# TonyLianLong/LLM-groundedDiffusion

Hardware: AMD Instinct MI355X
Metric: images/sec (50-step SD1.5 512^2, LMD+ guidance) (higher is better)
Workload: dtype fp16

## Files before the change

include/lgd_hip.h:

```cpp
#ifndef LGD_HIP_H
#define LGD_HIP_H
#include <stdint.h>
#ifdef __cplusplus
extern "C" {
#endif

#define LGD_ABI_VERSION 12
int lgd_abi_version(void);
int lgd_set_option(const char* name, int value);

#define LGD_EPI_GEGLU 1
#define LGD_EPI_OUT_F32 2
#define LGD_EPI_RES_F32 4
#define LGD_EPI_ROWNORM 8

typedef struct LgdGemmDesc {
  const void* a0;
  const void* a1;
  int64_t lda0, lda1;
  int32_t c0, c1;
  int32_t taps;
  int32_t hin, win, hout, wout, stride, ups;
  const void* w;
  int64_t ldw;
  int32_t M, N, K;
  int32_t nb_o, nb_i;
  int64_t a_bs_o, a_bs_i, w_bs_o, w_bs_i, c_bs_o, c_bs_i, r_bs_o, r_bs_i;
  const float* bias;
  const float* bias2;
  const void* res;
  int64_t ldr;
  float alpha;
  int32_t epi;
  void* c;
  int64_t ldc;
  int32_t splits;
  float* ws;
  int32_t tile;
  int32_t* cnt;
  const float* rowstat;
  const float* colsum;
} LgdGemmDesc;

int lgd_gemm_f16(const LgdGemmDesc* desc , void* stream);
int lgd_gemm_check(const LgdGemmDesc* desc );

int lgd_conv_in_f16(const float* x_nchw, const void* w, const float* bias, void* y, int B, int Cin,
                    int L, int Cout, void* stream);
int lgd_conv_out_f16(const void* x, const void* w, const float* bias, float* y_nchw, int B, int Cin,
                     int L, int Cout, float out_scale, void* stream);

int lgd_groupnorm_f16(const void* x0, const void* x1, int c0, int c1, int B, int HW, int G,
                      float eps, const float* gamma, const float* beta, int silu, void* y,
                      float* part, int nchunk, float* stats, void* stream);
int lgd_groupnorm_bwd_f16(const void* gy, const void* x0, const void* x1, int c0, int c1, int B,
                          int HW, int G, const float* gamma, const float* beta, int silu,
                          const float* stats, void* gx0, void* gx1, float* part, int nchunk,
                          int accumulate, void* stream);

int lgd_layernorm_f16(const void* x, int64_t ldx, void* y, int64_t ldy, int rows, int C, float eps,
                      const float* gamma, const float* beta, float* stats, int rows_per_batch,
                      int64_t x_bs, int64_t y_bs, void* stream);
int lgd_layernorm_bwd_f16(const void* gy, int64_t ldgy, const void* x, int64_t ldx, void* gx,
                          int64_t ldgx, int rows, int C, const float* gamma, const float* stats,
                          int rows_per_batch, int64_t gy_bs, int64_t x_bs, int64_t gx_bs,
                          int accumulate, void* stream);

int lgd_attn_fwd_f16(const void* q, int64_t ldq, int64_t q_bs, const void* k, int64_t ldk,
                     int64_t k_bs, const void* v, int64_t ldv, int64_t v_bs, void* o, int64_t ldo,
                     int64_t o_bs, float* lse, int B, int H, int Sq, int Sk, int d, float scale,
                     void* stream);
int lgd_attn_bwd_f16(const void* q, int64_t ldq, int64_t q_bs, const void* k, int64_t ldk,
                     int64_t k_bs, const void* v, int64_t ldv, int64_t v_bs, const void* o,
                     int64_t ldo, int64_t o_bs, const void* go, int64_t ldgo, int64_t go_bs,
                     const float* lse, float* delta, void* gq, int64_t ldgq, int64_t gq_bs, void* gk,
                     int64_t ldgk, int64_t gk_bs, void* gv, int64_t ldgv, int64_t gv_bs, int B, int H,
                     int Sq, int Sk, int d, float scale, void* stream);
int lgd_attn_bwd_keys_f16(const void* q, int64_t ldq, int64_t q_bs, const void* k, int64_t ldk,
                          int64_t k_bs, const void* v, int64_t ldv, int64_t v_bs, const void* o,
                          int64_t ldo, int64_t o_bs, const void* go, int64_t ldgo, int64_t go_bs,
                          const float* lse, float* delta, void* gq, int64_t ldgq, int64_t gq_bs, void* gk,
                          int64_t ldgk, int64_t gk_bs, void* gv, int64_t ldgv, int64_t gv_bs, int B, int H,
                          int Sq, int Sk, int Sk_grad, int d, float scale, void* stream);

int lgd_cross_attn_fwd_f16(const void* q, int64_t ldq, int64_t q_bs, const void* k, int64_t ldk,
                           int64_t k_bs, const void* v, int64_t ldv, int64_t v_bs, void* o,
                           int64_t ldo, int64_t o_bs, float* probs, int tok, int cond_only, int B,
                           int H, int Sq, int Sk, int d, float scale, void* stream);
int lgd_cross_attn_bwd_f16(const void* q, int64_t ldq, int64_t q_bs, const void* k, int64_t ldk,
                           int64_t k_bs, const void* v, int64_t ldv, int64_t v_bs, const void* go,
                           int64_t ldgo, int64_t go_bs, const float* gp, void* gq, int64_t ldgq,
                           int64_t gq_bs, int B, int H, int Sq, int Sk, int d, float scale,
                           void* stream);

int lgd_attn_causal_fwd_f16(const void* q, int64_t ldq, int64_t q_bs, const void* k, int64_t ldk, int64_t k_bs,
                            const void* v, int64_t ldv, int64_t v_bs, void* o, int64_t ldo, int64_t o_bs, int B,
                            int H, int S, int d, float scale, void* stream);

int lgd_geglu_bwd_f16(const void* h, const void* gy, void* gh, int64_t rows, int n, void* stream);
int lgd_geglu_fwd_f16(const void* h, void* y, int64_t rows, int n, void* stream);
int lgd_quick_gelu_f16(const void* x, void* y, int64_t n, void* stream);
int lgd_nchw_to_nhwc8_f16(const float* x, void* y, int B, int C, int HW, void* stream);
int lgd_add_f16(const void* a, const void* b, void* y, int64_t n, void* stream);
int lgd_scale_f16(const void* x, void* y, float alpha, int64_t n, void* stream);
int lgd_softmax_rows_f16(const void* x, void* y, int64_t rows, int n, float scale, void* stream);
int lgd_upsample2x_bwd_f16(const void* gy, void* gx, int B, int H, int W, int C, void* stream);

int lgd_cfg_ddim_step_f32(const float* eps, const float* x, float* x_out, const float* coef_table,
                          const int32_t* dyn, const float* frozen_ref, const float* mask, float* hist,
                          int B, int C, int HW, void* stream);
int lgd_cfg_multistep_step_f32(const float* eps, const float* x, float* x_out, float* x0_prev,
                               const float* coef_table, const int32_t* dyn, const float* frozen_ref,
                               const float* mask, float* hist, int B, int C, int HW, void* stream);
int lgd_cfg_plms_step_f32(const float* eps, const float* x, float* x_out, float* ets, float* cur_sample,
                          const float* coef_table, const int32_t* dyn, float* hist, int B, int C, int HW, void* stream);
int lgd_scale_rows_f32(const float* x, float* out, const float* table, const int32_t* dyn, int row_stride, int col,
                       int64_t n, int reps, void* stream);
int lgd_axpy_f32(const float* g, float* x, const float* coef_table, const int32_t* step_idx, int col,
                 const float* active, int64_t per_sample, int64_t n, void* stream);
int lgd_select_row_f32(const float* table, const int32_t* idx, float* out, int n, void* stream);

#define LGD_ACT_GELU 1
#define LGD_ACT_RELU 2
int lgd_act_f16(const void* x, void* y, int64_t n, int mode, void* stream);
int lgd_sam_relpos_qkv_f16(const void* qkv, const float* qkv_bias, const float* rel_h, const float* rel_w, int B,
                           int Hs, int Ws, int window, int NH, int d, int DA, float scale, void* qa, void* ka,
                           void* va, void* stream);
int lgd_sam_window_merge_f16(const void* oa, void* out, int B, int Hs, int Ws, int window, int NH, int d, int DA,
                             void* stream);

int lgd_ca_energy_f32(const float* const* maps, float* const* gmaps, const int32_t* map_hw,
                      const int32_t* items, const float* coefs, const float* masks, const float* refs,
                      int64_t refs_step_stride, const int32_t* dyn, const int32_t* groups, int n_groups,
                      int n_items, int n_samples, int H, int T, int max_hw, float grad_scale, float* partial,
                      float* loss, void* stream);

int lgd_boxdiff_energy_f32(const float* const* maps, float* const* gmaps, int n_maps, int side, const int32_t* items,
                           const float* masks, const float* smooth, const int32_t* groups, int n_samples,
                           int max_items, int H, int T, float loss_scale, float grad_scale, float* loss, void* stream);

#ifdef __cplusplus
}
#endif
#endif
```

llm-groundeddiffusion_amd/_lib.py:

```python
import ctypes as C
import os

import torch

_HERE = os.path.dirname(os.path.abspath(__file__))
LIB_PATH = os.path.join(_HERE, "liblgd_hip.so")
ABI_VERSION = 12

c_void_p, c_int, c_i64, c_float = C.c_void_p, C.c_int, C.c_int64, C.c_float


class LgdGemmDesc(C.Structure):
    _fields_ = [
        ("a0", c_void_p), ("a1", c_void_p),
        ("lda0", c_i64), ("lda1", c_i64),
        ("c0", C.c_int32), ("c1", C.c_int32),
        ("taps", C.c_int32),
        ("hin", C.c_int32), ("win", C.c_int32), ("hout", C.c_int32), ("wout", C.c_int32),
        ("stride", C.c_int32), ("ups", C.c_int32),
        ("w", c_void_p), ("ldw", c_i64),
        ("M", C.c_int32), ("N", C.c_int32), ("K", C.c_int32),
        ("nb_o", C.c_int32), ("nb_i", C.c_int32),
        ("a_bs_o", c_i64), ("a_bs_i", c_i64), ("w_bs_o", c_i64), ("w_bs_i", c_i64),
        ("c_bs_o", c_i64), ("c_bs_i", c_i64), ("r_bs_o", c_i64), ("r_bs_i", c_i64),
        ("bias", c_void_p), ("bias2", c_void_p),
        ("res", c_void_p), ("ldr", c_i64),
        ("alpha", c_float), ("epi", C.c_int32),
        ("c", c_void_p), ("ldc", c_i64),
        ("splits", C.c_int32), ("ws", c_void_p),
        ("tile", C.c_int32),
        ("cnt", c_void_p),
        ("rowstat", c_void_p), ("colsum", c_void_p),
    ]


EPI_GEGLU, EPI_OUT_F32, EPI_RES_F32, EPI_ROWNORM = 1, 2, 4, 8

_P, _I, _L, _F = c_void_p, c_int, c_i64, c_float
SIGNATURES = {
    "lgd_abi_version": [],
    "lgd_set_option": [C.c_char_p, _I],
    "lgd_gemm_f16": [C.POINTER(LgdGemmDesc), _P],
    "lgd_gemm_check": [C.POINTER(LgdGemmDesc)],
    "lgd_conv_in_f16": [_P, _P, _P, _P, _I, _I, _I, _I, _P],
    "lgd_conv_out_f16": [_P, _P, _P, _P, _I, _I, _I, _I, _F, _P],
    "lgd_groupnorm_f16": [_P, _P, _I, _I, _I, _I, _I, _F, _P, _P, _I, _P, _P, _I, _P, _P],
    "lgd_groupnorm_bwd_f16": [_P, _P, _P, _I, _I, _I, _I, _I, _P, _P, _I, _P, _P, _P, _P, _I, _I, _P],
    "lgd_layernorm_f16": [_P, _L, _P, _L, _I, _I, _F, _P, _P, _P, _I, _L, _L, _P],
    "lgd_layernorm_bwd_f16": [_P, _L, _P, _L, _P, _L, _I, _I, _P, _P, _I, _L, _L, _L, _I, _P],
    "lgd_attn_fwd_f16": [_P, _L, _L, _P, _L, _L, _P, _L, _L, _P, _L, _L, _P, _I, _I, _I, _I, _I, _F, _P],
    "lgd_attn_bwd_f16": [_P, _L, _L, _P, _L, _L, _P, _L, _L, _P, _L, _L, _P, _L, _L, _P, _P,
                         _P, _L, _L, _P, _L, _L, _P, _L, _L, _I, _I, _I, _I, _I, _F, _P],
    "lgd_attn_bwd_keys_f16": [_P, _L, _L, _P, _L, _L, _P, _L, _L, _P, _L, _L, _P, _L, _L, _P, _P,
                              _P, _L, _L, _P, _L, _L, _P, _L, _L, _I, _I, _I, _I, _I, _I, _F, _P],
    "lgd_cross_attn_fwd_f16": [_P, _L, _L, _P, _L, _L, _P, _L, _L, _P, _L, _L, _P, _I, _I,
                               _I, _I, _I, _I, _I, _F, _P],
    "lgd_cross_attn_bwd_f16": [_P, _L, _L, _P, _L, _L, _P, _L, _L, _P, _L, _L, _P, _P, _L, _L,
                               _I, _I, _I, _I, _I, _F, _P],
    "lgd_geglu_bwd_f16": [_P, _P, _P, _L, _I, _P],
    "lgd_geglu_fwd_f16": [_P, _P, _L, _I, _P],
    "lgd_add_f16": [_P, _P, _P, _L, _P],
    "lgd_softmax_rows_f16": [_P, _P, _L, _I, _F, _P],
    "lgd_scale_f16": [_P, _P, _F, _L, _P],
    "lgd_upsample2x_bwd_f16": [_P, _P, _I, _I, _I, _I, _P],
    "lgd_cfg_ddim_step_f32": [_P, _P, _P, _P, _P, _P, _P, _P, _I, _I, _I, _P],
    "lgd_cfg_multistep_step_f32": [_P, _P, _P, _P, _P, _P, _P, _P, _P, _I, _I, _I, _P],
    "lgd_cfg_plms_step_f32": [_P, _P, _P, _P, _P, _P, _P, _P, _I, _I, _I, _P],
    "lgd_axpy_f32": [_P, _P, _P, _P, _I, _P, _L, _L, _P],
    "lgd_select_row_f32": [_P, _P, _P, _I, _P],
    "lgd_scale_rows_f32": [_P, _P, _P, _P, _I, _I, _L, _I, _P],
    "lgd_attn_causal_fwd_f16": [_P, _L, _L, _P, _L, _L, _P, _L, _L, _P, _L, _L, _I, _I, _I, _I, _F, _P],
    "lgd_quick_gelu_f16": [_P, _P, _L, _P],
    "lgd_act_f16": [_P, _P, _L, _I, _P],
    "lgd_nchw_to_nhwc8_f16": [_P, _P, _I, _I, _I, _P],
    "lgd_sam_relpos_qkv_f16": [_P, _P, _P, _P, _I, _I, _I, _I, _I, _I, _I, _F, _P, _P, _P, _P],
    "lgd_sam_window_merge_f16": [_P, _P, _I, _I, _I, _I, _I, _I, _I, _P],
    "lgd_ca_energy_f32": [_P, _P, _P, _P, _P, _P, _P, _L, _P, _P, _I, _I, _I, _I, _I, _I, _F, _P, _P, _P],
    "lgd_boxdiff_energy_f32": [_P, _P, _I, _I, _P, _P, _P, _P, _I, _I, _I, _I, _F, _F, _P, _P],
}

_lib = None


def load():
    global _lib
    if _lib is not None:
        return _lib
    if not os.path.exists(LIB_PATH):
        raise RuntimeError(
            f"{LIB_PATH} not found: build it with `python __graft_entry__.py` "
            "(there is no CPU/PyTorch fallback for the HIP kernels)")
    lib = C.CDLL(LIB_PATH)
    for name, argtypes in SIGNATURES.items():
        try:
            fn = getattr(lib, name)
        except AttributeError as e:
            raise RuntimeError(f"liblgd_hip.so does not export {name}") from e
        fn.argtypes = argtypes
        fn.restype = c_int
    if lib.lgd_abi_version() != ABI_VERSION:
        raise RuntimeError("liblgd_hip.so ABI version mismatch; rebuild")
    for item in filter(None, os.environ.get("LGD_OPTIONS", "").split(",")):
        name, _, value = item.partition("=")
        check(lib.lgd_set_option(name.strip().encode(), int(value)), f"lgd_set_option({name})")
    _lib = lib
    return lib


_ERR = {-1: "invalid argument", -2: "kernel launch failed", -3: "unsupported shape"}


def check(rc, name):
    if rc != 0:
        raise RuntimeError(f"{name} failed: {_ERR.get(rc, rc)}")
```

llm-groundeddiffusion_amd/csrc/attn.hip:

```cpp
#include <atomic>
#include "common.h"
#include "../../include/lgd_hip.h"
#include "attn_w4.h"
#include <stdlib.h>
#include <string.h>

namespace {

int g_attn32_nw = -1;
int attn32_nw() {
  if (g_attn32_nw < 0) { const char* e = getenv("LGD_ATTN32_NW"); g_attn32_nw = e ? atoi(e) : 8; }
  return g_attn32_nw;
}
int g_attn32_var = 0;
int attn32_var() { return g_attn32_var; }
int g_attn32 = -1;
int attn32_mode() {
  if (g_attn32 < 0) { const char* e = getenv("LGD_ATTN32"); g_attn32 = e ? atoi(e) : 1; }
  return g_attn32;
}

std::atomic<int> g_attn_w4{-1};
int attn_w4_mode() {
  int v = g_attn_w4.load(std::memory_order_relaxed);
// ... 791 lines not shown
    __syncthreads();
    if (t + 2 < n_tiles) load_k((t + 2) * KV_T);
    if (more) load_v((t + 1) * KV_T);
    const float mx_nxt = pipelined_tile((t + 1) & 1, t & 1, s_cur, s_nxt);
    if (more) {
      const float mx = mx_nxt;
      if (__builtin_amdgcn_ballot_w64(mx > 8.f) != 0) {
        const float m_new = (float)(half_t)fmaxf(m_ref, mx + m_ref);
        const float shift = m_new - m_ref;
        const float alpha = __builtin_amdgcn_exp2f(-shift);
#pragma unroll
        for (int dt = 0; dt < NDT; ++dt)
#pragma unroll
          for (int r = 0; r < 16; ++r) oacc[dt][r] *= alpha;
#pragma unroll
        for (int kb = 0; kb < 2; ++kb)
#pragma unroll
          for (int r = 0; r < 16; ++r) s_nxt[kb][r] -= shift;
        m_ref = m_new;
        set_ref(m_new);
      }
#pragma unroll
      for (int kb = 0; kb < 2; ++kb) s_cur[kb] = s_nxt[kb];
    }
  }

  float l;
  {
    const int dl = d & 31, dt_l = d >> 5, h_l = (dl >> 2) & 1, r_l = (dl & 3) + 4 * (dl >> 3);
    float lv = 0.f;
#pragma unroll
    for (int dt = 0; dt < NDT; ++dt)
#pragma unroll
      for (int r = 0; r < 16; ++r)
        if (dt == dt_l && r == r_l) lv = oacc[dt][r];
    l = __shfl(lv, h_l * 32 + qi, 64);
  }
  const int qrow = q0 + qi;
  if (qrow < a.Sq) {
    const float inv = 1.f / l;
    half_t* orow = a.o + (long)b * a.o_bs + (long)qrow * a.ldo + (long)h * d;
#pragma unroll
    for (int dt = 0; dt < NDT; ++dt)
#pragma unroll
      for (int g4 = 0; g4 < 4; ++g4) {
        const int dv = dt * 32 + g4 * 8 + hh * 4;
        if (dv < d) {
          half4_t o;
#pragma unroll
          for (int r = 0; r < 4; ++r) o[r] = (half_t)(oacc[dt][g4 * 4 + r] * inv);
          *reinterpret_cast<half4_t*>(orow + dv) = o;
        }
      }
    if (a.lse && hh == 0) a.lse[((long)b * a.H + h) * a.Sq + qrow] = m_ref + log2f(l);
  }
}

template <int DP, bool SAVE_P>
void launch_attn_dp(const AttnArgs& a, hipStream_t st) {
  if constexpr (SAVE_P) {
    dim3 grid((a.Sq + 63) / 64, a.H, a.B);
    hipLaunchKernelGGL((attn_fwd_kernel<DP>), grid, dim3(256), 0, st, a);
  } else {
    if constexpr (DP == 64 || DP == 96) {
      const int a32 = attn32_mode();
      const int dk = ((a.d + 2 + 15) / 16) * 16;
      const long blocks256 = (long)((a.Sq + 255) / 256) * a.H * a.B;
      if (a32 && a.d % 8 == 0 && (a32 == 2 || (dk == 96 && blocks256 >= 128))) {
        const int var = attn32_var();
        auto go = [&](auto kern, int nw) {
          dim3 g32((a.Sq + 32 * nw - 1) / (32 * nw), a.H, a.B);
          hipLaunchKernelGGL(kern, g32, dim3(64 * nw), 0, st, a);
        };
        if (attn32_nw() == 4 || (a32 != 2 && blocks256 < 256)) {
          if (dk == 48) { go(&attn_self32_kernel<48, 2, 4>, 4); return; }
          if (dk == 96) { go(&attn_self32_kernel<96, 3, 4>, 4); return; }
        } else if (var == 1) {
          if (dk == 48) { go(&attn_self32_kernel<48, 2, 8, 4, true>, 8); return; }
          if (dk == 96) { go(&attn_self32_kernel<96, 3, 8, 4, true>, 8); return; }
        } else if (var == 2) {
          if (dk == 48) { go(&attn_self32_kernel<48, 2, 8, 2, false>, 8); return; }
          if (dk == 96) { go(&attn_self32_kernel<96, 3, 8, 2, false>, 8); return; }
        } else {
          if (dk == 48) { go(&attn_self32_kernel<48, 2, 8>, 8); return; }
          if (dk == 96) { go(&attn_self32_kernel<96, 3, 8>, 8); return; }
        }
      }
    }
    const bool qt2 = (long)((a.Sq + 127) / 128) * a.H * a.B >= 1024 && DP <= 96;
    dim3 grid(qt2 ? (a.Sq + 127) / 128 : (a.Sq + 63) / 64, a.H, a.B);
    if constexpr (DP <= 96) {
      static const int nw_env = [] { const char* e = getenv("LGD_ATTN_NW"); return e ? atoi(e) : 0; }();
      const bool nw8 = nw_env ? nw_env == 8 : ((DP == 64 && a.d < 48) || DP == 96);
      if (qt2 && nw8 && (long)((a.Sq + 255) / 256) * a.H * a.B >= 512) {
        dim3 g8((a.Sq + 255) / 256, a.H, a.B);
        if (DP == 64 && a.d < 48) hipLaunchKernelGGL((attn_self_kernel<DP, true, 2, DP == 64 ? 3 : DP / 16, 8>), g8, dim3(512), 0, st, a);
        else if (a.d < DP) hipLaunchKernelGGL((attn_self_kernel<DP, true, 2, DP / 16, 8>), g8, dim3(512), 0, st, a);
        else hipLaunchKernelGGL((attn_self_kernel<DP, false, 2, DP / 16, 8>), g8, dim3(512), 0, st, a);
        return;
      }
      if (qt2) {
        if (DP == 64 && a.d < 48) hipLaunchKernelGGL((attn_self_kernel<DP, true, 2, DP == 64 ? 3 : DP / 16>), grid, dim3(256), 0, st, a);
        else if (a.d < DP) hipLaunchKernelGGL((attn_self_kernel<DP, true, 2>), grid, dim3(256), 0, st, a);
        else hipLaunchKernelGGL((attn_self_kernel<DP, false, 2>), grid, dim3(256), 0, st, a);
        return;
      }
    }
    if constexpr (DP == 160) {
      static const int wide = [] { const char* e = getenv("LGD_ATTN160"); return e ? atoi(e) : 1; }();
      if (wide && a.d == DP && a.Sq >= 256 && (long)a.H * a.B * ((a.Sq + 63) / 64) > 256) {
        dim3 g8((a.Sq + 255) / 256, a.H, a.B);
        hipLaunchKernelGGL((attn_self_kernel<DP, false, 2, DP / 16, 8>), g8, dim3(512), 0, st, a);
        return;
      }
    }
    if (DP == 64 && a.d < 48) hipLaunchKernelGGL((attn_self_kernel<DP, true, 1, DP == 64 ? 3 : DP / 16>), grid, dim3(256), 0, st, a);
    else if (a.d < DP) hipLaunchKernelGGL((attn_self_kernel<DP, true, 1>), grid, dim3(256), 0, st, a);
    else hipLaunchKernelGGL((attn_self_kernel<DP, false, 1>), grid, dim3(256), 0, st, a);
  }
}

template <bool SAVE_P>
int launch_attn(const AttnArgs& a, hipStream_t st) {
  const int d = a.d;
  if constexpr (!SAVE_P) {
    const int w4 = attn_w4_mode();
    if (w4 && d == 40) {
      AttnW4Args w;
      w.q = a.q; w.ldq = a.ldq; w.q_bs = a.q_bs; w.k = a.k; w.ldk = a.ldk; w.k_bs = a.k_bs;
      w.v = a.v; w.ldv = a.ldv; w.v_bs = a.v_bs; w.o = a.o; w.ldo = a.ldo; w.o_bs = a.o_bs; w.lse = a.lse;
      w.B = a.B; w.H = a.H; w.Sq = a.Sq; w.Sk = a.Sk; w.d = a.d; w.scale_log2 = a.scale_log2;
      const long wgs = (long)((a.Sq + 255) / 256) * a.H * a.B;
      if (lgd_attn_w4_supported(w) && (w4 == 2 || (wgs >= 256 && a.Sk >= 256))) return lgd_attn_w4_launch(w, st);
    }
  }
  if (d <= 32) launch_attn_dp<32, SAVE_P>(a, st);
  else if (d <= 64) launch_attn_dp<64, SAVE_P>(a, st);
  else if (d <= 96) launch_attn_dp<96, SAVE_P>(a, st);
  else if (d <= 128) launch_attn_dp<128, SAVE_P>(a, st);
  else if (d <= 160) launch_attn_dp<160, SAVE_P>(a, st);
  else if (d <= 192) launch_attn_dp<192, SAVE_P>(a, st);
  else return LGD_ERR_UNSUPPORTED;
  return lgd_check_launch();
}

bool bad_view(int64_t ld, int d) { return (ld % 8) != 0 || (d % 8) != 0; }

}

void lgd_gn_set_fused_hw(int hw);
void lgd_gn_set_slab(int on);
void lgd_ln_set_stream(int on);
void lgd_gn_set_apply_wgs(int n);

extern "C" int lgd_set_option(const char* name, int value) {
  if (!name) return LGD_ERR_ARG;
  if (!strcmp(name, "gn_fused") && value >= 0 && value <= 4096) { lgd_gn_set_fused_hw(value); return LGD_OK; }
  if (!strcmp(name, "gn_slab") && (value == 0 || value == 1)) { lgd_gn_set_slab(value); return LGD_OK; }
  if (!strcmp(name, "ln_stream") && (value == 0 || value == 1)) { lgd_ln_set_stream(value); return LGD_OK; }
  if (!strcmp(name, "gn_apply_wgs") && value >= 64 && value <= 8192) { lgd_gn_set_apply_wgs(value); return LGD_OK; }
  if (!strcmp(name, "attn32")) { g_attn32 = value; return LGD_OK; }
  if (!strcmp(name, "attn_w4") && value >= 0 && value <= 2) { g_attn_w4.store(value, std::memory_order_relaxed); return LGD_OK; }
  if (!strcmp(name, "attn_w4_pipe") && (value == 0 || value == 1)) { lgd_attn_w4_set_pipe(value); return LGD_OK; }
  if (!strcmp(name, "attn32_nw") && (value == 4 || value == 8)) { g_attn32_nw = value; return LGD_OK; }
  if (!strcmp(name, "attn32_var") && value >= 0 && value <= 2) { g_attn32_var = value; return LGD_OK; }
  return LGD_ERR_ARG;
}

extern "C" int lgd_attn_fwd_f16(const void* q, int64_t ldq, int64_t q_bs, const void* k,
                                int64_t ldk, int64_t k_bs, const void* v, int64_t ldv, int64_t v_bs,
                                void* o, int64_t ldo, int64_t o_bs, float* lse, int B, int H, int Sq,
                                int Sk, int d, float scale, void* stream) {
  (void)hipGetLastError();
  if (B < 1 || H < 1 || Sq < 1 || Sk < 1 || d < 8) return LGD_ERR_ARG;
  if (bad_view(ldq, d) || bad_view(ldk, d) || bad_view(ldv, d) || (ldo % 4)) return LGD_ERR_ARG;
  AttnArgs a;
  a.q = (const half_t*)q; a.ldq = ldq; a.q_bs = q_bs;
  a.k = (const half_t*)k; a.ldk = ldk; a.k_bs = k_bs;
  a.v = (const half_t*)v; a.ldv = ldv; a.v_bs = v_bs;
  a.o = (half_t*)o; a.ldo = ldo; a.o_bs = o_bs;
  a.lse = lse; a.probs = nullptr; a.tok = -1; a.cond_only = 0; a.causal = 0;
  a.B = B; a.H = H; a.Sq = Sq; a.Sk = Sk; a.d = d;
  a.scale_log2 = scale * 1.4426950408889634f;
  return launch_attn<false>(a, reinterpret_cast<hipStream_t>(stream));
}

extern "C" int lgd_cross_attn_fwd_f16(const void* q, int64_t ldq, int64_t q_bs, const void* k,
                                      int64_t ldk, int64_t k_bs, const void* v, int64_t ldv,
                                      int64_t v_bs, void* o, int64_t ldo, int64_t o_bs, float* probs,
                                      int tok, int cond_only, int B, int H, int Sq, int Sk, int d,
                                      float scale, void* stream) {
  (void)hipGetLastError();
  if (B < 1 || H < 1 || Sq < 1 || Sk < 1 || d < 8) return LGD_ERR_ARG;
  if (bad_view(ldq, d) || bad_view(ldk, d) || bad_view(ldv, d) || (ldo % 4)) return LGD_ERR_ARG;
  if (cond_only && (B % 2)) return LGD_ERR_ARG;
  if (tok >= Sk) return LGD_ERR_ARG;
  AttnArgs a;
  a.q = (const half_t*)q; a.ldq = ldq; a.q_bs = q_bs;
  a.k = (const half_t*)k; a.ldk = ldk; a.k_bs = k_bs;
  a.v = (const half_t*)v; a.ldv = ldv; a.v_bs = v_bs;
  a.o = (half_t*)o; a.ldo = ldo; a.o_bs = o_bs;
  a.lse = nullptr; a.probs = probs; a.tok = tok; a.cond_only = cond_only; a.causal = 0;
  a.B = B; a.H = H; a.Sq = Sq; a.Sk = Sk; a.d = d;
  a.scale_log2 = scale * 1.4426950408889634f;
  hipStream_t st = reinterpret_cast<hipStream_t>(stream);
  if (probs) return launch_attn<true>(a, st);
  return launch_attn<false>(a, st);
}

extern "C" int lgd_attn_causal_fwd_f16(const void* q, int64_t ldq, int64_t q_bs, const void* k, int64_t ldk,
                                       int64_t k_bs, const void* v, int64_t ldv, int64_t v_bs, void* o,
                                       int64_t ldo, int64_t o_bs, int B, int H, int S, int d, float scale,
                                       void* stream) {
  (void)hipGetLastError();
  if (B < 1 || H < 1 || S < 1 || d < 8) return LGD_ERR_ARG;
  if (bad_view(ldq, d) || bad_view(ldk, d) || bad_view(ldv, d) || (ldo % 4)) return LGD_ERR_ARG;
  AttnArgs a;
  a.q = (const half_t*)q; a.ldq = ldq; a.q_bs = q_bs;
  a.k = (const half_t*)k; a.ldk = ldk; a.k_bs = k_bs;
  a.v = (const half_t*)v; a.ldv = ldv; a.v_bs = v_bs;
  a.o = (half_t*)o; a.ldo = ldo; a.o_bs = o_bs;
  a.lse = nullptr; a.probs = nullptr; a.tok = -1; a.cond_only = 0; a.causal = 1;
  a.B = B; a.H = H; a.Sq = S; a.Sk = S; a.d = d;
  a.scale_log2 = scale * 1.4426950408889634f;
  return launch_attn<true>(a, reinterpret_cast<hipStream_t>(stream));
}
```

llm-groundeddiffusion_amd/csrc/gemm.hip:

```cpp
#include "common.h"
#include "../../include/lgd_hip.h"
#include <map>
#include <mutex>
#include <utility>
#include <stdlib.h>

namespace {

constexpr int BK = 64;
constexpr int LDS_LD = BK + 16;

struct GemmArgs {
  LgdGemmDesc d;
  int cin;
  int k_per_split;
  int group_m;
#ifdef LGD_GEMM_ABLATION
  int stagger;
#endif
};

__device__ __forceinline__ float4 ld_bias4(const float* p, int n) {
  return *reinterpret_cast<const float4*>(p + n);
}

__device__ __forceinline__ f32x4 rownorm4(const LgdGemmDesc& d, int m, int n_in, f32x4 v) {
  if (d.epi & LGD_EPI_ROWNORM) {
    const float2 st = *reinterpret_cast<const float2*>(d.rowstat + (long)m * 2);
    const float4 cs = *reinterpret_cast<const float4*>(d.colsum + n_in);
    v[0] = st.y * (v[0] - st.x * cs.x); v[1] = st.y * (v[1] - st.x * cs.y);
    v[2] = st.y * (v[2] - st.x * cs.z); v[3] = st.y * (v[3] - st.x * cs.w);
  }
  return v;
}

template <bool GEGLU>
__device__ __forceinline__ f32x4 epilogue_value4(const LgdGemmDesc& d, long r_off, int m, int n_out, f32x4 v, f32x4 g,
                                                 float4 bv, float4 bg, bool res_ready, half4_t res_pre) {
  v[0] += bv.x; v[1] += bv.y; v[2] += bv.z; v[3] += bv.w;
  if (GEGLU) {
    g[0] += bg.x; g[1] += bg.y; g[2] += bg.z; g[3] += bg.w;
#ifdef LGD_GEMM_ABLATION
    if (d.epi & (1 << 16)) {
#pragma unroll
      for (int r = 0; r < 4; ++r) v[r] = v[r] * g[r];
    } else
#endif
    {
      const f32x2_t g01 = gelu2_f((f32x2_t){g[0], g[1]}), g23 = gelu2_f((f32x2_t){g[2], g[3]});
      v[0] *= g01[0]; v[1] *= g01[1]; v[2] *= g23[0]; v[3] *= g23[1];
    }
  }
  const float alpha = d.alpha;
#pragma unroll
  for (int r = 0; r < 4; ++r) v[r] *= alpha;
  if (res_ready) {
#pragma unroll
    for (int r = 0; r < 4; ++r) v[r] += (float)res_pre[r];
  } else if (d.res) {
    if (d.epi & LGD_EPI_RES_F32) {
      const float* rp = reinterpret_cast<const float*>(d.res) + r_off + (long)m * d.ldr + n_out;
      float4 rv = *reinterpret_cast<const float4*>(rp);
      v[0] += rv.x; v[1] += rv.y; v[2] += rv.z; v[3] += rv.w;
    } else {
      const half_t* rp = reinterpret_cast<const half_t*>(d.res) + r_off + (long)m * d.ldr + n_out;
      half4_t rv = *reinterpret_cast<const half4_t*>(rp);
#pragma unroll
      for (int r = 0; r < 4; ++r) v[r] += (float)rv[r];
    }
  }
  return v;
}

template <bool GEGLU>
__device__ __forceinline__ void epilogue_store4(const LgdGemmDesc& d, long c_off, long r_off, int m,
                                                int n_out, f32x4 v, f32x4 g, float4 bv, float4 bg,
                                                bool res_ready = false,
                                                half4_t res_pre = (half4_t){0, 0, 0, 0}) {
  v = epilogue_value4<GEGLU>(d, r_off, m, n_out, v, g, bv, bg, res_ready, res_pre);
  if (d.epi & LGD_EPI_OUT_F32) {
    float* cp = reinterpret_cast<float*>(d.c) + c_off + (long)m * d.ldc + n_out;
    *reinterpret_cast<float4*>(cp) = make_float4(v[0], v[1], v[2], v[3]);
  } else {
    half_t* cp = reinterpret_cast<half_t*>(d.c) + c_off + (long)m * d.ldc + n_out;
    half4_t o;
#pragma unroll
    for (int r = 0; r < 4; ++r) o[r] = (half_t)v[r];
    *reinterpret_cast<half4_t*>(cp) = o;
  }
}

__device__ __forceinline__ float4 ld_bias_sum4(const LgdGemmDesc& d, int n) {
  float4 b = make_float4(0.f, 0.f, 0.f, 0.f);
  if (d.bias) b = ld_bias4(d.bias, n);
  if (d.bias2) {
    float4 b2 = ld_bias4(d.bias2, n);
    b.x += b2.x; b.y += b2.y; b.z += b2.z; b.w += b2.w;
  }
  return b;
}

template <int MI, int NI>
__device__ __forceinline__ void gemm_epilogue(const GemmArgs& ga, f32x4 (&acc)[NI][MI], int m0, int n0,
                                              int wm, int wn, int lane, int batch, int split,
                                              long c_off, long r_off, int* lds_flag = nullptr) {
  const LgdGemmDesc& d = ga.d;
  const int m_l = lane & 15;
  const int n_l = (lane >> 4) * 4;
  if (d.splits > 1) {
    float* ws = ga.d.ws + ((long)batch * d.splits + split) * (long)d.M * d.N;
#pragma unroll
    for (int mi = 0; mi < MI; ++mi) {
      int m = m0 + wm * 16 * MI + mi * 16 + m_l;
      if (m >= d.M) continue;
#pragma unroll
      for (int ni = 0; ni < NI; ++ni) {
        int n = n0 + wn * 16 * NI + ni * 16 + n_l;
        if (n >= d.N) continue;
        f32x4 v = acc[ni][mi];
        *reinterpret_cast<float4*>(ws + (long)m * d.N + n) = make_float4(v[0], v[1], v[2], v[3]);
      }
    }
    if (!d.cnt || !lds_flag) return;
    asm volatile("s_waitcnt vmcnt(0)" ::: "memory");
    __syncthreads();
    int32_t* cnt = d.cnt + (long)batch * gridDim.x + blockIdx.x;
    if (threadIdx.x == 0) {
      __builtin_amdgcn_fence(__ATOMIC_RELEASE, "agent");
      asm volatile("s_waitcnt vmcnt(0)" ::: "memory");
      *lds_flag = __hip_atomic_fetch_add(cnt, 1, __ATOMIC_RELAXED, __HIP_MEMORY_SCOPE_AGENT);
    }
    __syncthreads();
    if (*lds_flag != d.splits - 1) return;
    if (threadIdx.x == 0) {
      __builtin_amdgcn_fence(__ATOMIC_ACQUIRE, "agent");
      __hip_atomic_store(cnt, 0, __ATOMIC_RELAXED, __HIP_MEMORY_SCOPE_AGENT);
    }
    __syncthreads();
    const float* w0 = ga.d.ws + (long)batch * d.splits * (long)d.M * d.N;
#pragma unroll
    for (int mi = 0; mi < MI; ++mi) {
      const int m = m0 + wm * 16 * MI + mi * 16 + m_l;
#pragma unroll
      for (int ni = 0; ni < NI; ++ni) {
        const int n = n0 + wn * 16 * NI + ni * 16 + n_l;
        f32x4 v = {0.f, 0.f, 0.f, 0.f};
        if (m < d.M && n < d.N) {
          for (int s2 = 0; s2 < d.splits; ++s2) {
            const float4 t = *reinterpret_cast<const float4*>(w0 + (long)s2 * d.M * d.N + (long)m * d.N + n);
            v[0] += t.x; v[1] += t.y; v[2] += t.z; v[3] += t.w;
          }
        }
        acc[ni][mi] = v;
      }
    }
  }
  const bool geglu = d.epi & LGD_EPI_GEGLU;
  if (geglu) {
    if constexpr (NI % 2 == 0) {
#pragma unroll
      for (int ni = 0; ni < NI; ni += 2) {
        const int n_in = n0 + wn * 16 * NI + ni * 16 + n_l;
        if (n_in >= d.N) continue;
        const int n_out = (n0 + wn * 16 * NI + ni * 16) / 2 + n_l;
        const float4 bv = ld_bias_sum4(d, n_in);
        float4 bg = make_float4(0.f, 0.f, 0.f, 0.f);
        if (d.bias) bg = ld_bias4(d.bias, n_in + 16);
#pragma unroll
        for (int mi = 0; mi < MI; ++mi) {
// ... 14 lines not shown
    half4_t rpre[NCH][MI];
    if (res16) {
      const half_t* rb = reinterpret_cast<const half_t*>(d.res) + r_off;
#pragma unroll
      for (int nj = 0; nj < NCH; ++nj) {
        int n = n0 + wn * 16 * NI + (nc + nj) * 16 + n_l;
        if (n >= d.N) n = 0;
#pragma unroll
        for (int mi = 0; mi < MI; ++mi) {
          int m = m0 + wm * 16 * MI + mi * 16 + m_l;
          if (m >= d.M) m = d.M - 1;
          rpre[nj][mi] = *reinterpret_cast<const half4_t*>(rb + (long)m * d.ldr + n);
        }
      }
    }
#pragma unroll
    for (int nj = 0; nj < NCH; ++nj) {
      const int ni = nc + nj;
      const int n = n0 + wn * 16 * NI + ni * 16 + n_l;
      if (n >= d.N) continue;
      const float4 bv = ld_bias_sum4(d, n);
#pragma unroll
      for (int mi = 0; mi < MI; ++mi) {
        const int m = m0 + wm * 16 * MI + mi * 16 + m_l;
        if (m < d.M)
          epilogue_store4<false>(d, c_off, r_off, m, n, rownorm4(d, m, n, acc[ni][mi]), acc[ni][mi], bv, bv, res16,
                                 res16 ? rpre[nj][mi] : (half4_t){0, 0, 0, 0});
      }
    }
  }
}

template <int MI, int NI, int WM, int WN, int STAGE_B, bool GEGLU, bool RES_PREFETCH>
__device__ __forceinline__ void gemm_epilogue_lds_generic(const GemmArgs& ga, f32x4 (&acc)[NI][MI], int m0, int n0, int wm,
                                                  int wn, int lane, int tid, long c_off, long r_off,
                                                  unsigned char* lds) {
  const LgdGemmDesc& d = ga.d;
  constexpr int NT = 64 * WM * WN;
  constexpr int BM = WM * 16 * MI, BN = WN * 16 * NI;
  constexpr int BN_OUT = GEGLU ? BN / 2 : BN;
  constexpr int NI_OUT = GEGLU ? NI / 2 : NI;
  constexpr int CROW = BN_OUT * 2 + 16;
  constexpr int R = (BM * CROW <= STAGE_B) ? 1 : ((BM / 2) * CROW <= STAGE_B) ? 2 : 4;
  static_assert(MI % R == 0 && (BM / R) * CROW <= STAGE_B, "staged rows must fit one ring stage");
  constexpr int MI_R = MI / R;
  constexpr int WROWS = 16 * MI_R;
  constexpr int RROWS = WM * WROWS;
  constexpr int CPR = BN_OUT / 8;
  const int m_l = lane & 15, n_l = (lane >> 4) * 4;
  const int n0_out = GEGLU ? n0 / 2 : n0;
  const int n_total_out = GEGLU ? d.N / 2 : d.N;
  const bool res16 = d.res && !(d.epi & LGD_EPI_RES_F32);
  half_t* cbase = reinterpret_cast<half_t*>(d.c) + c_off;
  float4 bv[NI_OUT], bg[NI_OUT];
  const bool rn = d.epi & LGD_EPI_ROWNORM;
  float4 cv[NI_OUT], cg[NI_OUT];
  float2 st[MI];
#pragma unroll
  for (int no = 0; no < NI_OUT; ++no) {
    const int n_out = n0_out + wn * 16 * NI_OUT + no * 16 + n_l;
    const int n_in = GEGLU ? n0 + wn * 16 * NI + no * 32 + n_l : n_out;
    bv[no] = make_float4(0.f, 0.f, 0.f, 0.f);
    bg[no] = bv[no];
    cv[no] = bv[no];
    cg[no] = bv[no];
#ifdef LGD_GEMM_ABLATION
    if (d.epi & (1 << 18)) continue;
#endif
    if (n_out < n_total_out) {
      bv[no] = ld_bias_sum4(d, n_in);
      if (GEGLU && d.bias) bg[no] = ld_bias4(d.bias, n_in + 16);
      if (rn) {
        cv[no] = *reinterpret_cast<const float4*>(d.colsum + n_in);
        if (GEGLU) cg[no] = *reinterpret_cast<const float4*>(d.colsum + n_in + 16);
      }
    }
  }
#pragma unroll
  for (int mi = 0; mi < MI; ++mi) {
    int m = m0 + wm * 16 * MI + mi * 16 + m_l;
    if (m >= d.M) m = d.M - 1;
    st[mi] = rn ? *reinterpret_cast<const float2*>(d.rowstat + (long)m * 2) : make_float2(0.f, 1.f);
  }
  auto rownorm = [&](f32x4 v, const float2 s2, const float4 c) {
    if (rn) {
      v[0] = s2.y * (v[0] - s2.x * c.x); v[1] = s2.y * (v[1] - s2.x * c.y);
      v[2] = s2.y * (v[2] - s2.x * c.z); v[3] = s2.y * (v[3] - s2.x * c.w);
    }
    return v;
  };
#pragma unroll
  for (int r = 0; r < R; ++r) {
    half4_t rpre[NI_OUT][MI_R];
    if (res16 && !GEGLU) {
      const half_t* rb = reinterpret_cast<const half_t*>(d.res) + r_off;
#pragma unroll
      for (int no = 0; no < NI_OUT; ++no) {
        int n = n0_out + wn * 16 * NI_OUT + no * 16 + n_l;
        if (n >= n_total_out) n = 0;
#pragma unroll
        for (int mj = 0; mj < MI_R; ++mj) {
          int m = m0 + wm * 16 * MI + (r * MI_R + mj) * 16 + m_l;
          if (m >= d.M) m = d.M - 1;
          rpre[no][mj] = *reinterpret_cast<const half4_t*>(rb + (long)m * d.ldr + n);
        }
      }
    }
#pragma unroll
    for (int no = 0; no < NI_OUT; ++no) {
      const int n_out = n0_out + wn * 16 * NI_OUT + no * 16 + n_l;
      const int nn = n_out < n_total_out ? n_out : 0;
#pragma unroll
      for (int mj = 0; mj < MI_R; ++mj) {
        const int mi = r * MI_R + mj;
        int m = m0 + wm * 16 * MI + mi * 16 + m_l;
        if (m >= d.M) m = d.M - 1;
        f32x4 v;
        if constexpr (GEGLU) {
          v = epilogue_value4<true>(d, r_off, m, nn, rownorm(acc[2 * no][mi], st[mi], cv[no]), rownorm(acc[2 * no + 1][mi], st[mi], cg[no]),
                                    bv[no], bg[no], false, (half4_t){0, 0, 0, 0});
        } else {
          v = epilogue_value4<false>(d, r_off, m, nn, rownorm(acc[no][mi], st[mi], cv[no]), acc[no][mi], bv[no], bv[no], res16,
                                     res16 ? rpre[no][mj] : (half4_t){0, 0, 0, 0});
        }
        half4_t o;
#pragma unroll
        for (int e = 0; e < 4; ++e) o[e] = (half_t)v[e];
        *reinterpret_cast<half4_t*>(lds + (wm * WROWS + mj * 16 + m_l) * CROW + (wn * 16 * NI_OUT + no * 16 + n_l) * 2) = o;
      }
    }
    asm volatile("s_waitcnt lgkmcnt(0)" ::: "memory");
    __builtin_amdgcn_s_barrier();
#pragma unroll
    for (int i = 0; i < (RROWS * CPR + NT - 1) / NT; ++i) {
      const int idx = tid + i * NT;
      const int row = idx / CPR, ch = idx - row * CPR;
      const int wr = row / WROWS;
      const int m = m0 + wr * 16 * MI + r * WROWS + (row - wr * WROWS), n = n0_out + ch * 8;
#ifdef LGD_GEMM_ABLATION
      if ((d.epi & (1 << 17)) && idx != 0) continue;
#endif
      if (idx < RROWS * CPR && m < d.M && n < n_total_out) {
        const uint4 val = *reinterpret_cast<const uint4*>(lds + row * CROW + ch * 16);
        *reinterpret_cast<uint4*>(cbase + (long)m * d.ldc + n) = val;
      }
    }
    if (r + 1 < R || !RES_PREFETCH) {
      asm volatile("s_waitcnt lgkmcnt(0)" ::: "memory");
      __builtin_amdgcn_s_barrier();
    }
  }
}

template <int MI, int NI, int WM, int WN, int STAGE_B, bool GEGLU, bool RES_PREFETCH, bool RES16, bool RN>
__device__ __forceinline__ void gemm_epilogue_lds(const GemmArgs& ga, f32x4 (&acc)[NI][MI], int m0, int n0, int wm,
                                                  int wn, int lane, int tid, long c_off, long r_off,
                                                  unsigned char* lds) {
  static_assert(!(GEGLU && RES16), "GEGLU outputs take no residual here");
  const LgdGemmDesc& d = ga.d;
  constexpr int NT = 64 * WM * WN;
  constexpr int BM = WM * 16 * MI, BN = WN * 16 * NI;
  constexpr int BN_OUT = GEGLU ? BN / 2 : BN;
  constexpr int NI_OUT = GEGLU ? NI / 2 : NI;
  constexpr int CROW = BN_OUT * 2 + 16;
  constexpr int R = (BM * CROW <= STAGE_B) ? 1 : ((BM / 2) * CROW <= STAGE_B) ? 2 : 4;
  static_assert(MI % R == 0 && (BM / R) * CROW <= STAGE_B, "staged rows must fit one ring stage");
  constexpr int MI_R = MI / R;
  constexpr int WROWS = 16 * MI_R;
  constexpr int RROWS = WM * WROWS;
  constexpr int CPR = BN_OUT / 8;
  const int m_l = lane & 15, n_l = (lane >> 4) * 4;
  const int n0_out = GEGLU ? n0 / 2 : n0;
  const int n_total_out = GEGLU ? d.N / 2 : d.N;
  half_t* cbase = reinterpret_cast<half_t*>(d.c) + c_off;
  const f32x2_t alpha2 = {d.alpha, d.alpha};
  constexpr bool LEAN = MI * NI >= 32;
  constexpr bool LEAN2 = MI * NI >= 32 && WN == 4;
  float4 bv[NI_OUT], bg[NI_OUT], cv[NI_OUT], cg[NI_OUT];
  int ncol[NI_OUT];
#pragma unroll
  for (int no = 0; no < NI_OUT; ++no) {
    const int n_out = n0_out + wn * 16 * NI_OUT + no * 16 + n_l;
    const int n_in = GEGLU ? n0 + wn * 16 * NI + no * 32 + n_l : n_out;
    const bool ok = n_out < n_total_out;
    ncol[no] = ok ? n_out : 0;
    bv[no] = make_float4(0.f, 0.f, 0.f, 0.f);
    bg[no] = bv[no];
    cv[no] = bv[no];
    cg[no] = bv[no];
#ifdef LGD_GEMM_ABLATION
    if (d.epi & (1 << 18)) continue;
#endif
    if (ok && !LEAN2) {
      bv[no] = ld_bias_sum4(d, n_in);
      if (GEGLU && d.bias) bg[no] = ld_bias4(d.bias, n_in + 16);
      if constexpr (RN && !LEAN) {
        cv[no] = *reinterpret_cast<const float4*>(d.colsum + n_in);
        if (GEGLU) cg[no] = *reinterpret_cast<const float4*>(d.colsum + n_in + 16);
      }
    }
  }
  int mrow[MI];
  float2 st[MI];
#pragma unroll
  for (int mi = 0; mi < MI; ++mi) {
    int m = m0 + wm * 16 * MI + mi * 16 + m_l;
    if (m >= d.M) m = d.M - 1;
    mrow[mi] = m;
    st[mi] = make_float2(0.f, 1.f);
    if constexpr (RN && !LEAN2) st[mi] = *reinterpret_cast<const float2*>(d.rowstat + (long)m * 2);
  }
  auto normed = [&](const f32x4& v, const float2 s2, const float4 c, const float4 b, f32x2_t& lo, f32x2_t& hi) {
    lo = (f32x2_t){v[0], v[1]};
    hi = (f32x2_t){v[2], v[3]};
    if constexpr (RN) {
      const f32x2_t mean = {s2.x, s2.x}, rstd = {s2.y, s2.y};
      lo = rstd * (lo - mean * (f32x2_t){c.x, c.y});
      hi = rstd * (hi - mean * (f32x2_t){c.z, c.w});
    }
    lo += (f32x2_t){b.x, b.y};
    hi += (f32x2_t){b.z, b.w};
  };
  unsigned char* lw = lds + (wm * WROWS + m_l) * CROW + (wn * 16 * NI_OUT + n_l) * 2;
#pragma unroll
  for (int r = 0; r < R; ++r) {
    if constexpr (RN && LEAN2) {
#pragma unroll
      for (int mj = 0; mj < MI_R; ++mj)
        st[r * MI_R + mj] = *reinterpret_cast<const float2*>(d.rowstat + (long)mrow[r * MI_R + mj] * 2);
    }
    half4_t rpre[NI_OUT][MI_R];
    if constexpr (RES16) {
      const half_t* rb = reinterpret_cast<const half_t*>(d.res) + r_off;
#pragma unroll
      for (int mj = 0; mj < MI_R; ++mj) {
        const half_t* rrow = rb + (long)mrow[r * MI_R + mj] * d.ldr;
#pragma unroll
        for (int no = 0; no < NI_OUT; ++no) {
          int nc = ncol[no];
          if constexpr (LEAN) {
            const int n_out = n0_out + wn * 16 * NI_OUT + no * 16 + n_l;
            nc = n_out < n_total_out ? n_out : 0;
          }
          rpre[no][mj] = *reinterpret_cast<const half4_t*>(rrow + nc);
        }
      }
    }
#pragma unroll
    for (int no = 0; no < NI_OUT; ++no) {
      if constexpr ((RN && LEAN) || LEAN2) {
        const int n_out = n0_out + wn * 16 * NI_OUT + no * 16 + n_l;
        const int n_in = GEGLU ? n0 + wn * 16 * NI + no * 32 + n_l : n_out;
        if (n_out < n_total_out) {
          if constexpr (RN) {
            cv[no] = *reinterpret_cast<const float4*>(d.colsum + n_in);
            if (GEGLU) cg[no] = *reinterpret_cast<const float4*>(d.colsum + n_in + 16);
          }
          if constexpr (LEAN2) {
            bv[no] = ld_bias_sum4(d, n_in);
            if (GEGLU && d.bias) bg[no] = ld_bias4(d.bias, n_in + 16);
          }
        }
      }
#pragma unroll
      for (int mj = 0; mj < MI_R; ++mj) {
        const int mi = r * MI_R + mj;
        f32x2_t lo, hi;
        if constexpr (GEGLU) {
          f32x2_t glo, ghi;
          normed(acc[2 * no][mi], st[mi], cv[no], bv[no], lo, hi);
          normed(acc[2 * no + 1][mi], st[mi], cg[no], bg[no], glo, ghi);
#ifdef LGD_GEMM_ABLATION
          if (d.epi & (1 << 16)) { lo *= glo; hi *= ghi; } else
#endif
          { lo *= gelu2_f(glo); hi *= gelu2_f(ghi); }
        } else {
          normed(acc[no][mi], st[mi], cv[no], bv[no], lo, hi);
        }
        lo *= alpha2;
        hi *= alpha2;
        if constexpr (RES16) {
          const half4_t rr = rpre[no][mj];
          lo += (f32x2_t){(float)rr[0], (float)rr[1]};
          hi += (f32x2_t){(float)rr[2], (float)rr[3]};
        }
        const half4_t o = {(half_t)lo[0], (half_t)lo[1], (half_t)hi[0], (half_t)hi[1]};
        *reinterpret_cast<half4_t*>(lw + mj * 16 * CROW + no * 32) = o;
      }
    }
    asm volatile("s_waitcnt lgkmcnt(0)" ::: "memory");
    __builtin_amdgcn_s_barrier();
#pragma unroll LEAN2 ? 1 : (RROWS * CPR + NT - 1) / NT
    for (int i = 0; i < (RROWS * CPR + NT - 1) / NT; ++i) {
      const int idx = tid + i * NT;
      const int row = idx / CPR, ch = idx - row * CPR;
      const int wr = row / WROWS;
      const int m = m0 + wr * 16 * MI + r * WROWS + (row - wr * WROWS), n = n0_out + ch * 8;
#ifdef LGD_GEMM_ABLATION
      if ((d.epi & (1 << 17)) && idx != 0) continue;
#endif
      if (idx < RROWS * CPR && m < d.M && n < n_total_out) {
        const uint4 val = *reinterpret_cast<const uint4*>(lds + row * CROW + ch * 16);
        *reinterpret_cast<uint4*>(cbase + (long)m * d.ldc + n) = val;
      }
    }
    if (r + 1 < R || !RES_PREFETCH) {
      asm volatile("s_waitcnt lgkmcnt(0)" ::: "memory");
      __builtin_amdgcn_s_barrier();
    }
  }
}

template <int MI, int NI>
__global__ __launch_bounds__(256) void gemm_kernel(const GemmArgs ga) {
  constexpr int BM = 32 * MI;
  constexpr int BN = 32 * NI;
  constexpr int A_IT = BM * 8 / 256;
  constexpr int B_IT = BN * 8 / 256;
  static_assert(A_IT >= 1 && B_IT >= 1, "tile too small");

  __shared__ __attribute__((aligned(16))) half_t smem[(BM + BN) * LDS_LD];
  half_t* As = smem;
  half_t* Bs = smem + BM * LDS_LD;

  const LgdGemmDesc& d = ga.d;
  const int tid = threadIdx.x;
  const int lane = tid & 63;
  const int wid = tid >> 6;
  const int wm = wid >> 1, wn = wid & 1;

  const int n_tiles_n = (d.N + BN - 1) / BN;
  const int tile_m = blockIdx.x / n_tiles_n;
  const int tile_n = blockIdx.x - tile_m * n_tiles_n;
  const int zz = blockIdx.z;
  const int batch = zz / d.splits;
  const int split = zz - batch * d.splits;
  const int b_o = batch / d.nb_i, b_i = batch - b_o * d.nb_i;
  const long a_off = b_o * d.a_bs_o + b_i * d.a_bs_i;
  const long w_off = b_o * d.w_bs_o + b_i * d.w_bs_i;
  const long c_off = b_o * d.c_bs_o + b_i * d.c_bs_i;
  const long r_off = b_o * d.r_bs_o + b_i * d.r_bs_i;

  const int m0 = tile_m * BM, n0 = tile_n * BN;
  const int k_beg = split * ga.k_per_split;
  int k_end = k_beg + ga.k_per_split;
  if (k_end > d.K) k_end = d.K;
  const int nk = (k_end - k_beg + BK - 1) / BK;

  const half_t* A0 = reinterpret_cast<const half_t*>(d.a0) + a_off;
  const half_t* A1 = d.a1 ? reinterpret_cast<const half_t*>(d.a1) + a_off : nullptr;
  const half_t* W = reinterpret_cast<const half_t*>(d.w) + w_off;

  const int kseg = tid & 7;
  const int rbase = tid >> 3;
  const int cin = ga.cin;
  const bool conv = d.taps == 9;

  int a_iy0[A_IT], a_ix0[A_IT];
  long a_row[A_IT];
  bool a_ok[A_IT];
#pragma unroll
  for (int i = 0; i < A_IT; ++i) {
    int m = m0 + rbase + 32 * i;
    a_ok[i] = m < d.M;
    if (conv) {
      int hw = d.hout * d.wout;
      int b = m / hw;
      int rem = m - b * hw;
      int oy = rem / d.wout;
      int ox = rem - oy * d.wout;
      a_iy0[i] = oy * d.stride - 1;
      a_ix0[i] = ox * d.stride - 1;
      a_row[i] = (long)b * d.hin * d.win;
    } else {
      a_iy0[i] = 0; a_ix0[i] = 0;
      a_row[i] = m;
    }
  }
  int k_cur = k_beg + kseg * 8;
  int tap = conv ? k_cur / cin : 0;
  int ch = k_cur - tap * cin;

  uint4 a_reg[A_IT], b_reg[B_IT];

  auto load_tile = [&]() {
    const bool k_ok = k_cur < k_end;
    int ky = 0, kx = 0;
    if (conv) { ky = tap / 3; kx = tap - ky * 3; }
    const bool src1 = ch >= d.c0;
    const half_t* src = src1 ? A1 : A0;
    const long ld = src1 ? d.lda1 : d.lda0;
    const int cc = src1 ? ch - d.c0 : ch;
#pragma unroll
    for (int i = 0; i < A_IT; ++i) {
      bool ok = a_ok[i] && k_ok;
      long row = a_row[i];
      if (conv) {
        int iy = a_iy0[i] + ky, ix = a_ix0[i] + kx;
        if (d.ups) {
          ok = ok && iy >= 0 && ix >= 0 && iy < 2 * d.hin && ix < 2 * d.win;
          if (d.ups == 2) ok = ok && !((iy | ix) & 1);
          iy >>= 1; ix >>= 1;
        } else {
          ok = ok && iy >= 0 && ix >= 0 && iy < d.hin && ix < d.win;
        }
        row += (long)iy * d.win + ix;
      }
      if (ok) a_reg[i] = *reinterpret_cast<const uint4*>(src + row * ld + cc);
      else a_reg[i] = make_uint4(0, 0, 0, 0);
    }
#pragma unroll
    for (int i = 0; i < B_IT; ++i) {
      int n = n0 + rbase + 32 * i;
      bool ok = (n < d.N) && k_ok;
      if (ok) b_reg[i] = *reinterpret_cast<const uint4*>(W + (long)n * d.ldw + k_cur);
      else b_reg[i] = make_uint4(0, 0, 0, 0);
    }
    k_cur += BK;
    ch += BK;
    if (conv) {
      while (ch >= cin) { ch -= cin; ++tap; }
    }
  };
  auto store_tile = [&]() {
#pragma unroll
    for (int i = 0; i < A_IT; ++i)
      *reinterpret_cast<uint4*>(As + (rbase + 32 * i) * LDS_LD + kseg * 8) = a_reg[i];
#pragma unroll
    for (int i = 0; i < B_IT; ++i)
      *reinterpret_cast<uint4*>(Bs + (rbase + 32 * i) * LDS_LD + kseg * 8) = b_reg[i];
  };

  f32x4 acc[NI][MI];
#pragma unroll
  for (int ni = 0; ni < NI; ++ni)
#pragma unroll
    for (int mi = 0; mi < MI; ++mi) acc[ni][mi] = (f32x4){0.f, 0.f, 0.f, 0.f};

  const int frow = lane & 15;
  const int fk = (lane >> 4) * 8;

  if (nk > 0) {
    load_tile();
    store_tile();
    __syncthreads();
    for (int kt = 0; kt < nk; ++kt) {
      if (kt + 1 < nk) load_tile();
#pragma unroll
      for (int kk = 0; kk < BK / 32; ++kk) {
        half8_t af[MI], bf[NI];
#pragma unroll
        for (int mi = 0; mi < MI; ++mi)
          af[mi] = *reinterpret_cast<const half8_t*>(
              As + (wm * 16 * MI + mi * 16 + frow) * LDS_LD + kk * 32 + fk);
#pragma unroll
        for (int ni = 0; ni < NI; ++ni)
          bf[ni] = *reinterpret_cast<const half8_t*>(
              Bs + (wn * 16 * NI + ni * 16 + frow) * LDS_LD + kk * 32 + fk);
#pragma unroll
        for (int ni = 0; ni < NI; ++ni)
#pragma unroll
// ... 440 lines not shown
      else p = (a_ok[j] && live) ? a_ptr[j] : zero;
      __builtin_amdgcn_global_load_lds((glb_ptr_t)p, (lds_ptr_t)(As + (j * NW + wid) * 8 * BK), 16, 0, 0);
    } else {
      const int i = j - A_IT;
      const half_t* p = live ? w_row[i] : zero;
      if (B_HALF && i == B_FULL) {
        if (b_half_on)
          __builtin_amdgcn_global_load_lds((glb_ptr_t)p, (lds_ptr_t)(Bs + b_grp_last * 8 * BK), 16, 0, 0);
      } else {
        __builtin_amdgcn_global_load_lds((glb_ptr_t)p, (lds_ptr_t)(Bs + (i * NW + wid) * 8 * BK), 16, 0, 0);
      }
    }
  };
  auto advance = [&]() {
    ++kt_issue;
    if constexpr (TWO) return;
    if (CM) {
      int wstep = cin;
      if (++tap0 == 9) { tap0 = 0; ch0 += BK; wstep = BK - 8 * cin; }
#pragma unroll
      for (int i = 0; i < B_IT; ++i) w_row[i] += wstep;
      cm_offset();
    } else {
#pragma unroll
      for (int i = 0; i < B_IT; ++i) w_row[i] += BK;
#pragma unroll
      for (int i = 0; i < A_IT; ++i) a_ptr[i] += BK;
      const int prev = ch0;
      ch0 += BK;
      bool red = prev < d.c0 && ch0 >= d.c0;
      if (ch0 >= cin) { ch0 -= cin; ++tap0; red = true; }
      if (red && kt_issue < nk) derive();
    }
  };

  f32x4 acc[NI][MI];
#pragma unroll
  for (int ni = 0; ni < NI; ++ni)
#pragma unroll
    for (int mi = 0; mi < MI; ++mi) acc[ni][mi] = (f32x4){0.f, 0.f, 0.f, 0.f};

  const int frow = lane & 15;
  const int fg = lane >> 4;
  const int fsw = (frow >> 1) & 7;
  const unsigned lds0 = (unsigned)(uintptr_t)smem;
  const unsigned a_b0 = lds0 + ((wm * 16 * MI + frow) * BK + ((0 * 4 + fg) ^ fsw) * 8) * 2;
  const unsigned a_b1 = lds0 + ((wm * 16 * MI + frow) * BK + ((1 * 4 + fg) ^ fsw) * 8) * 2;
  constexpr int B_OFF = BM * BK * 2;
  const unsigned b_b0 = a_b0 - (wm * 16 * MI) * BK * 2 + B_OFF + (wn * 16 * NI) * BK * 2;
  const unsigned b_b1 = a_b1 - (wm * 16 * MI) * BK * 2 + B_OFF + (wn * 16 * NI) * BK * 2;
  using seqA = std::make_integer_sequence<int, MI>;
  using seqB = std::make_integer_sequence<int, NI>;
  constexpr int FSTR = 16 * BK * 2;

  half8_t af0[MI], bf0[NI], af1[MI], bf1[NI];
  auto mma_range = [&](half8_t (&af)[MI], half8_t (&bf)[NI], int g0, int g1) {
#pragma unroll
    for (int g = 0; g < NMMA; ++g)
      if (g >= g0 && g < g1) {
        const int ni = g / MI, mi = g % MI;
        if constexpr (ABL & 4) {
          asm volatile("" : "+v"(acc[ni][mi]) : "v"(bf[ni]), "v"(af[mi]));
        } else {
          acc[ni][mi] = __builtin_amdgcn_mfma_f32_16x16x32_f16(bf[ni], af[mi], acc[ni][mi], 0, 0, 0);
        }
      }
  };
  auto dma_and_mma = [&](int j0, int cnt, unsigned so_b, bool live, half8_t (&af)[MI], half8_t (&bf)[NI]) {
#pragma unroll
    for (int j = 0; j < T_DMA; ++j)
      if (j < cnt) {
        if constexpr (!(ABL & 1)) issue_one(j0 + j, (int)(so_b >> 1), live);
        __builtin_amdgcn_sched_barrier(0);
        mma_range(af, bf, (NMMA * j) / cnt, (NMMA * (j + 1)) / cnt);
        __builtin_amdgcn_sched_barrier(0);
      }
    if (cnt == 0) mma_range(af, bf, 0, NMMA);
  };

  int v_issue = blockIdx.x;
  bool issue_dead = false;
  auto begin_k_tile = [&]() {
    if constexpr (!PERSIST) {
      issue_dead = kt_issue >= nk;
      return;
    }
    if (kt_issue >= nk && !issue_dead) {
      v_issue += gridDim.x;
      if (v_issue < total_tiles) {
        int m0n, n0n;
        tile_origin(v_issue, m0n, n0n);
        setup_issue(m0n, n0n);
        if (CM) cm_offset(); else derive();
      } else {
        issue_dead = true;
      }
    }
  };

  if (nk > 0) {
    int m0, n0;
    tile_origin(blockIdx.x, m0, n0);
    setup_issue(m0, n0);
    if (CM) cm_offset(); else derive();
#pragma unroll
    for (int t = 0; t < D; ++t) {
      begin_k_tile();
#pragma unroll
      for (int j = 0; j < T_DMA; ++j) issue_one(j, t * STAGE, !issue_dead);
      advance();
    }
    asm volatile("s_waitcnt vmcnt(%0)" ::"n"((D - 1) * T_DMA) : "memory");
    __builtin_amdgcn_s_barrier();
    lds_read_frags<0, FSTR>(af0, a_b0, seqA{});
    lds_read_frags<0, FSTR>(bf0, b_b0, seqB{});
    unsigned so_cur = 0, so_nxt = STAGE_B, so_iss = (D % NS) * STAGE_B;
    auto next_stage = [](unsigned x) { x += STAGE_B; return x == NS * STAGE_B ? 0u : x; };
    auto k_loop = [&]() {
      for (int kt = 0; kt < nk; ++kt) {
        begin_k_tile();
        const bool live = !issue_dead;
        wait_frags<-1>(af0, bf0);
        if constexpr (!(ABL & 2)) {
          lds_read_frags<0, FSTR>(af1, a_b1 + so_cur, seqA{});
          lds_read_frags<0, FSTR>(bf1, b_b1 + so_cur, seqB{});
        }
        dma_and_mma(0, T1, so_iss, live, af0, bf0);
        wait_frags<(D - 2) * T_DMA + T1>(af1, bf1);
        if constexpr (!(ABL & 8)) __builtin_amdgcn_s_barrier();
        if constexpr (!(ABL & 2)) {
          if (!PERSIST || kt + 1 < nk) {
            lds_read_frags<0, FSTR>(af0, a_b0 + so_nxt, seqA{});
            lds_read_frags<0, FSTR>(bf0, b_b0 + so_nxt, seqB{});
          }
        }
        dma_and_mma(T1, T2, so_iss, live, af1, bf1);
        advance();
        so_cur = so_nxt; so_nxt = next_stage(so_nxt); so_iss = next_stage(so_iss);
      }
    };
    const bool lds_epi = d.splits == 1 && !(d.epi & LGD_EPI_OUT_F32) && !(d.N & 7) && !(d.ldc & 7) && !(c_off & 7) &&
                         !(reinterpret_cast<uintptr_t>(d.c) & 15) && !((d.epi & LGD_EPI_GEGLU) && (NI & 1)) &&
                         !(d.res && (d.epi & (LGD_EPI_RES_F32 | LGD_EPI_GEGLU)));
    auto epilogue = [&](int m0_, int n0_) {
      if constexpr (ABL & 16) {
#pragma unroll
        for (int ni = 0; ni < NI; ++ni)
#pragma unroll
          for (int mi = 0; mi < MI; ++mi) asm volatile("" ::"v"(acc[ni][mi]));
        return;
      }
      if (lds_epi) {
        unsigned char* free_stage = reinterpret_cast<unsigned char*>(smem) + so_iss;
#define LGD_EPI_LDS(G, RS, RNORM) \
  gemm_epilogue_lds<MI, NI, WM, WN, STAGE_B, G, !PERSIST, RS, RNORM>(ga, acc, m0_, n0_, wm, wn, lane, tid, c_off, r_off, free_stage)
        const bool rn_ = d.epi & LGD_EPI_ROWNORM;
        if constexpr (MI * NI >= 32) {
          if (d.epi & LGD_EPI_GEGLU)
            gemm_epilogue_lds_generic<MI, NI, WM, WN, STAGE_B, true, !PERSIST>(ga, acc, m0_, n0_, wm, wn, lane, tid, c_off, r_off, free_stage);
          else
            gemm_epilogue_lds_generic<MI, NI, WM, WN, STAGE_B, false, !PERSIST>(ga, acc, m0_, n0_, wm, wn, lane, tid, c_off, r_off, free_stage);
        } else if (d.epi & LGD_EPI_GEGLU) {
          if constexpr (NI % 2 == 0) {
            if (rn_) LGD_EPI_LDS(true, false, true); else LGD_EPI_LDS(true, false, false);
          }
        } else if (d.res) {
          if (rn_) LGD_EPI_LDS(false, true, true); else LGD_EPI_LDS(false, true, false);
        } else {
          if (rn_) LGD_EPI_LDS(false, false, true); else LGD_EPI_LDS(false, false, false);
        }
#undef LGD_EPI_LDS
      } else {
        if constexpr (!(TWO && MI * NI >= 32))
          gemm_epilogue<MI, NI>(ga, acc, m0_, n0_, wm, wn, lane, batch, split, c_off, r_off, reinterpret_cast<int*>(smem));
      }
    };
    if constexpr (PERSIST) {
      for (int v = blockIdx.x; v < total_tiles; v += gridDim.x) {
        tile_origin(v, m0, n0);
        k_loop();
        epilogue(m0, n0);
#pragma unroll
        for (int ni = 0; ni < NI; ++ni)
#pragma unroll
          for (int mi = 0; mi < MI; ++mi) acc[ni][mi] = (f32x4){0.f, 0.f, 0.f, 0.f};
        if constexpr (!(ABL & 2)) {
          lds_read_frags<0, FSTR>(af0, a_b0 + so_cur, seqA{});
          lds_read_frags<0, FSTR>(bf0, b_b0 + so_cur, seqB{});
        }
      }
      asm volatile("s_waitcnt vmcnt(0) lgkmcnt(0)" ::: "memory");
    } else {
      k_loop();
      asm volatile("s_waitcnt vmcnt(0) lgkmcnt(0)" ::: "memory");
      epilogue(m0, n0);
    }
  } else {
    for (int v = blockIdx.x; v < total_tiles; v += gridDim.x) {
      int m0, n0;
      tile_origin(v, m0, n0);
      if constexpr (!(TWO && MI * NI >= 32))
        gemm_epilogue<MI, NI>(ga, acc, m0, n0, wm, wn, lane, batch, split, c_off, r_off, reinterpret_cast<int*>(smem));
    }
  }
}

template <int MI, int NI, bool CM, int ABL = 0>
__global__ __launch_bounds__(512, 1) void gemm_phase_kernel(const GemmArgs ga) {
  constexpr int WM = 2, WN = 4;
  static_assert(MI == 8, "128 rows per wave group");
  constexpr int MH = MI / 2;
  constexpr int NI0 = (NI + 1) / 2, NI1 = NI - NI0;
  constexpr int BM = WM * 16 * MI, BN = WN * 16 * NI;
  constexpr int AQ_B = 2 * 16 * MH * 128;
  constexpr int BQ0_B = 64 * NI0 * 128, BQ1_B = 64 * NI1 * 128;
  constexpr int OFF_A1 = AQ_B, OFF_B0 = 2 * AQ_B, OFF_B1 = 2 * AQ_B + BQ0_B;
  constexpr int STAGE_B = 2 * AQ_B + BQ0_B + BQ1_B;
  static_assert(STAGE_B == (BM + BN) * BK * 2 && 2 * STAGE_B <= 160 * 1024, "LDS");
  constexpr int NA = 2;
  constexpr int T_DMA = 2 * NA + NI;
  constexpr unsigned OOB = 0x80000000u;
  constexpr unsigned NREC = 0x80000000u;

  extern __shared__ __attribute__((aligned(1024))) half_t smem[];
  unsigned char* lds = reinterpret_cast<unsigned char*>(smem);

  const LgdGemmDesc& d = ga.d;
  const int tid = threadIdx.x;
  const int lane = tid & 63;
  const int wid = __builtin_amdgcn_readfirstlane(tid >> 6);
  const int grp = wid >> 2, wn = wid & 3;

  const int n_tiles_n = (d.N + BN - 1) / BN;
  const int total_tiles = ((d.M + BM - 1) / BM) * n_tiles_n;
  int m0, n0;
  {
    const int q = total_tiles >> 3, r = total_tiles & 7;
    const int xcd = blockIdx.x & 7, idx = blockIdx.x >> 3;
    const int bid = (xcd < r ? xcd * (q + 1) : r * (q + 1) + (xcd - r) * q) + idx;
    int tile_m, tile_n;
    if (ga.group_m > 1) {
      const int per_group = ga.group_m * n_tiles_n;
      const int g = bid / per_group, in = bid - g * per_group;
      const int n_tiles_m = total_tiles / n_tiles_n;
      int rows = n_tiles_m - g * ga.group_m;
      if (rows > ga.group_m) rows = ga.group_m;
      tile_n = in / rows;
      tile_m = g * ga.group_m + (in - tile_n * rows);
    } else {
      tile_m = bid / n_tiles_n;
      tile_n = bid - tile_m * n_tiles_n;
    }
    m0 = __builtin_amdgcn_readfirstlane(tile_m * BM);
    n0 = __builtin_amdgcn_readfirstlane(tile_n * BN);
  }
  const int split = blockIdx.z;
  constexpr int batch = 0;
  constexpr long a_off = 0, w_off = 0, c_off = 0, r_off = 0;

  const int k_beg = split * ga.k_per_split;
  int k_end = k_beg + ga.k_per_split;
  if (k_end > d.K) k_end = d.K;
  const int nk = __builtin_amdgcn_readfirstlane((k_end - k_beg) / BK);
  const int cin = ga.cin;

  const int lrow = lane >> 3;
  const int kseg = (lane & 7) ^ ((((wid & 1) << 2) + (lrow >> 1)) & 7);
  const unsigned lda2 = (unsigned)d.lda0 * 2u, ldw2 = (unsigned)d.ldw * 2u;
  const int arow = wid * 8 + lrow;
  const int bcol = (wid >> 1) * 16 * NI + (wid & 1) * 8 + lrow;
  const half_t* a_base = reinterpret_cast<const half_t*>(d.a0) + a_off - (CM ? (long)(d.win + 1) * d.lda0 : 0L);
  const half_t* w_base = reinterpret_cast<const half_t*>(d.w) + w_off;
  const unsigned voffA = (unsigned)(m0 + arow) * lda2 + kseg * 16;
  const unsigned voffB = (unsigned)(n0 + bcol) * ldw2 + kseg * 16;
  unsigned amask[2] = {0u, 0u};
#pragma unroll
  for (int h = 0; h < 2; ++h)
#pragma unroll
    for (int j = 0; j < NA; ++j) {
      const int m = m0 + j * 128 + h * 16 * MH + arow;
      if (m >= d.M) continue;
      if (CM) {
        const int ox = m % d.wout, oy = (m / d.wout) % d.hout;
#pragma unroll
        for (int t = 0; t < 9; ++t) {
          const int iy = oy + t / 3 - 1, ix = ox + t % 3 - 1;
          if (iy >= 0 && ix >= 0 && iy < d.hin && ix < d.win) amask[h] |= 1u << (9 * j + t);
        }
      } else {
        amask[h] |= 1u << (9 * j);
      }
    }
  unsigned bmask = 0;
#pragma unroll
  for (int i = 0; i < NI; ++i)
    if (n0 + bcol + i * 16 < d.N) bmask |= 1u << i;

  const int t0 = k_beg / BK;
  auto k_pos = [&](int kt, unsigned& sa, unsigned& sw, int& tap) {
    if (CM) {
      const int t = t0 + kt, ch = __builtin_amdgcn_readfirstlane(t / 9);
      tap = t - ch * 9;
      const int ky = tap / 3, kx = tap - ky * 3;
      sa = (unsigned)(ky * d.win + kx) * lda2 + (unsigned)ch * (BK * 2);
      sw = (unsigned)(tap * cin + ch * BK) * 2u;
    } else {
      tap = 0;
      sa = sw = (unsigned)(k_beg + kt * BK) * 2u;
    }
  };
  auto dma_a = [&](int h, unsigned so, bool live, unsigned sa, int tap, bool inloop = true) {
    if ((ABL & 1) && inloop) return;
    const __amdgpu_buffer_rsrc_t rs = __builtin_amdgcn_make_buffer_rsrc(const_cast<half_t*>(a_base), 0, live ? NREC : 0u, 0x00020000);
#pragma unroll
    for (int j = 0; j < NA; ++j) {
      const unsigned vo = ((amask[h] >> (9 * j + tap)) & 1u) ? voffA : OOB;
      __builtin_amdgcn_raw_ptr_buffer_load_lds(rs, (lds_ptr_t)(lds + so + (h ? OFF_A1 : 0) + (j * 8 + wid) * 1024), 16, vo,
                                               sa + (unsigned)(j * 128 + h * 16 * MH) * lda2, 0, 0);
    }
  };
  auto dma_b = [&](int q, unsigned so, bool live, unsigned sw, bool inloop = true) {
    if ((ABL & 1) && inloop) return;
// ... 88 lines not shown
      LGD_PH_BAR();
      if constexpr (!(ABL & 2)) lds_read_frags<BQ0_B, 64 * 128>(bf1[0], b_ad0, seqB1{});
      if constexpr (!(ABL & 2)) lds_read_frags<BQ0_B, 64 * 128>(bf1[1], b_ad1, seqB1{});
      dma_a(1, so_nxt, live1, sa1, tap1);
      asm volatile("s_waitcnt vmcnt(%0)" ::"n"(T_DMA) : "memory");
      LGD_PH_BAR();
      LGD_PH_MMA(bf1, NI1, NI0, 0);
      LGD_PH_BAR();
      if constexpr (!(ABL & 2)) lds_read_frags<OFF_A1, 16 * 128>(af[0], a_ad0, seqA{});
      if constexpr (!(ABL & 2)) lds_read_frags<OFF_A1, 16 * 128>(af[1], a_ad1, seqA{});
      dma_b(0, so_cur, live2, sw2);
      LGD_PH_BAR();
      LGD_PH_MMA(bf1, NI1, NI0, MH);
      LGD_PH_BAR();
      dma_a(0, so_cur, live2, sa2, tap2);
      asm volatile("s_waitcnt vmcnt(%0)" ::"n"(T_DMA) : "memory");
      LGD_PH_BAR();
      LGD_PH_MMA(bf0, NI0, 0, MH);
      LGD_PH_BAR();
      a_ad0 += sdelta; a_ad1 += sdelta; b_ad0 += sdelta; b_ad1 += sdelta;
      sdelta = -sdelta;
      const unsigned t = so_cur; so_cur = so_nxt; so_nxt = t;
    }
    if (grp == 0 && !(ABL & 64)) LGD_PH_BAR();
    asm volatile("s_waitcnt vmcnt(0) lgkmcnt(0)" ::: "memory");
    LGD_PH_BAR();
  }
  else {
#pragma unroll
    for (int ni = 0; ni < NI; ++ni)
#pragma unroll
      for (int mi = 0; mi < MI; ++mi) acc[ni][mi] = (f32x4){0.f, 0.f, 0.f, 0.f};
  }
#undef LGD_PH_MMA
#undef LGD_PH_BAR

  if constexpr (ABL & 16) {
#pragma unroll
    for (int ni = 0; ni < NI; ++ni)
#pragma unroll
      for (int mi = 0; mi < MI; ++mi) asm volatile("" ::"v"(acc[ni][mi]));
    return;
  }
  if (d.splits > 1) {
    const int m_l = lane & 15, n_l = (lane >> 4) * 4;
    float* ws = d.ws + ((long)batch * d.splits + split) * (long)d.M * d.N;
#pragma unroll
    for (int mi = 0; mi < MI; ++mi) {
      const int m = m0 + grp * 16 * MI + mi * 16 + m_l;
      if (m >= d.M) continue;
#pragma unroll
      for (int ni = 0; ni < NI; ++ni) {
        const int n = n0 + wn * 16 * NI + ni * 16 + n_l;
        if (n >= d.N) continue;
        const f32x4 v = acc[ni][mi];
        *reinterpret_cast<float4*>(ws + (long)m * d.N + n) = make_float4(v[0], v[1], v[2], v[3]);
      }
    }
    return;
  }
#define LGD_EPI_LDS(G, RS, RNORM) \
  gemm_epilogue_lds<MI, NI, WM, WN, (MI * NI > 32 ? STAGE_B : 2 * STAGE_B), G, true, RS, RNORM>(ga, acc, m0, n0, grp, wn, lane, tid, c_off, r_off, lds)
  const bool rn_ = d.epi & LGD_EPI_ROWNORM;
  if (d.epi & LGD_EPI_GEGLU) {
    if constexpr (NI % 2 == 0) {
      if (rn_) LGD_EPI_LDS(true, false, true); else LGD_EPI_LDS(true, false, false);
    }
  } else if (d.res) {
    if (rn_) LGD_EPI_LDS(false, true, true); else LGD_EPI_LDS(false, true, false);
  } else {
    if (rn_) LGD_EPI_LDS(false, false, true); else LGD_EPI_LDS(false, false, false);
  }
#undef LGD_EPI_LDS
}

__global__ __launch_bounds__(256) void splitk_reduce_kernel(const GemmArgs ga) {
  const LgdGemmDesc& d = ga.d;
  const bool geglu = d.epi & LGD_EPI_GEGLU;
  const int n_out_cols = geglu ? d.N / 2 : d.N;
  const long groups_per_row = n_out_cols / 4;
  const long total = (long)d.M * groups_per_row;
  const int batch = blockIdx.z;
  const int b_o = batch / d.nb_i, b_i = batch - b_o * d.nb_i;
  const long c_off = b_o * d.c_bs_o + b_i * d.c_bs_i;
  const long r_off = b_o * d.r_bs_o + b_i * d.r_bs_i;
  const float* ws = d.ws + (long)batch * d.splits * (long)d.M * d.N;
  for (long idx = blockIdx.x * 256L + threadIdx.x; idx < total; idx += (long)gridDim.x * 256L) {
    int m = (int)(idx / groups_per_row);
    int gcol = (int)(idx - (long)m * groups_per_row) * 4;
    int n_in = geglu ? (gcol / 16) * 32 + (gcol % 16) : gcol;
    f32x4 v = {0.f, 0.f, 0.f, 0.f}, g = {0.f, 0.f, 0.f, 0.f};
    for (int s = 0; s < d.splits; ++s) {
      const float* p = ws + (long)s * d.M * d.N + (long)m * d.N + n_in;
      float4 t = *reinterpret_cast<const float4*>(p);
      v[0] += t.x; v[1] += t.y; v[2] += t.z; v[3] += t.w;
      if (geglu) {
        float4 u = *reinterpret_cast<const float4*>(p + 16);
        g[0] += u.x; g[1] += u.y; g[2] += u.z; g[3] += u.w;
      }
    }
    const float4 bv = ld_bias_sum4(d, n_in);
    v = rownorm4(d, m, n_in, v);
    if (geglu) {
      float4 bg = make_float4(0.f, 0.f, 0.f, 0.f);
      if (d.bias) bg = ld_bias4(d.bias, n_in + 16);
      epilogue_store4<true>(d, c_off, r_off, m, gcol, v, rownorm4(d, m, n_in + 16, g), bv, bg);
    } else {
      epilogue_store4<false>(d, c_off, r_off, m, gcol, v, g, bv, bv);
    }
  }
}

enum GemmLoop : int {
  LOOP_REG,
  LOOP_DMA,
  LOOP_DMA8,
  LOOP_PIPE,
  LOOP_PHASE,
};
enum : unsigned {
  TILE_GEGLU = 1,
  TILE_PLAIN = 2,
  TILE_ONE_SPLIT = 4,
  TILE_LDS_EPI = 8,
  TILE_CONV_SAME = 16,
  TILE_CNT = 32,
};
struct GemmTile {
  int code;
  GemmLoop loop;
  int bm, bn;
  unsigned flags;
};
constexpr unsigned TILE_STD = TILE_GEGLU | TILE_CNT;
constexpr GemmTile GEMM_TILES[] = {
    {1, LOOP_REG, 128, 128, TILE_STD},   {2, LOOP_REG, 128, 64, TILE_STD},     {3, LOOP_REG, 64, 128, TILE_STD},
    {4, LOOP_REG, 64, 64, TILE_STD},     {5, LOOP_REG, 32, 128, TILE_STD},     {6, LOOP_REG, 128, 160, TILE_CNT},
    {7, LOOP_REG, 64, 160, TILE_CNT},
    {17, LOOP_DMA, 128, 128, TILE_STD},  {18, LOOP_DMA, 128, 64, TILE_STD},    {19, LOOP_DMA, 64, 128, TILE_STD},
    {20, LOOP_DMA, 64, 64, TILE_STD},    {21, LOOP_DMA, 32, 128, TILE_STD},    {22, LOOP_DMA, 128, 160, TILE_CNT},
    {23, LOOP_DMA, 64, 160, TILE_CNT},
    {25, LOOP_DMA8, 256, 320, TILE_CNT}, {26, LOOP_DMA8, 256, 128, TILE_STD},
    {33, LOOP_PIPE, 256, 160, TILE_CNT}, {34, LOOP_PIPE, 256, 128, TILE_STD}, {35, LOOP_PIPE, 256, 64, TILE_STD},
    {37, LOOP_PIPE, 128, 160, TILE_CNT}, {38, LOOP_PIPE, 128, 128, TILE_STD}, {39, LOOP_PIPE, 128, 64, TILE_STD},
    {40, LOOP_PIPE, 64, 160, TILE_CNT},  {41, LOOP_PIPE, 64, 128, TILE_STD},  {42, LOOP_PIPE, 64, 64, TILE_STD},
    {44, LOOP_PIPE, 256, 256, TILE_GEGLU | TILE_PLAIN | TILE_ONE_SPLIT | TILE_LDS_EPI},
    {45, LOOP_PIPE, 128, 128, TILE_STD | TILE_PLAIN},
    {46, LOOP_PHASE, 256, 256, TILE_GEGLU | TILE_LDS_EPI | TILE_CONV_SAME},
    {47, LOOP_PHASE, 256, 320, TILE_LDS_EPI | TILE_CONV_SAME},
};

const GemmTile* gemm_check(const LgdGemmDesc& desc, GemmArgs& ga) {
  ga.d = desc;
  LgdGemmDesc& d = ga.d;
  if (d.M <= 0 || d.N <= 0 || d.K <= 0) return nullptr;
  if (d.taps != 1 && d.taps != 9) return nullptr;
  ga.cin = d.c0 + d.c1;
  if (d.K != d.taps * ga.cin) return nullptr;
  if ((d.c0 % 8) || (d.c1 % 8) || (d.N % 4) || (d.ldw % 8) || (d.lda0 % 8) || (d.lda1 % 8) ||
      (d.ldc % 4))
    return nullptr;
  if (d.c1 > 0 && !d.a1) return nullptr;
  if (d.res && (d.ldr % 4)) return nullptr;
  if (d.nb_o < 1) d.nb_o = 1;
  if (d.nb_i < 1) d.nb_i = 1;
  if (d.splits < 1) d.splits = 1;
  const bool geglu = d.epi & LGD_EPI_GEGLU;
  if (geglu && (d.N % 32)) return nullptr;
  if (d.splits > 1 && !d.ws) return nullptr;
  if ((d.epi & LGD_EPI_ROWNORM) && (!d.rowstat || !d.colsum || d.taps != 1 || d.nb_o * d.nb_i != 1 || d.c1 > 0))
    return nullptr;
  int ktiles = (d.K + BK - 1) / BK;
  int tps = (ktiles + d.splits - 1) / d.splits;
  ga.k_per_split = tps * BK;
  d.splits = (ktiles + tps - 1) / tps;

  int code = d.tile;
  if (code == 0) {
    long batches = (long)d.nb_o * d.nb_i * d.splits;
    auto wgs = [&](int bm, int bn) {
      return batches * ((d.M + bm - 1) / bm) * ((d.N + bn - 1) / bn);
    };
    if (d.M <= 32) code = 21;
    else if (!geglu && d.N % 160 == 0 && wgs(128, 160) >= 384) code = 22;
    else if (!geglu && d.N % 160 == 0 && wgs(64, 160) >= 256) code = 23;
    else if (wgs(128, 128) >= 384 && d.N % 128 == 0) code = 17;
    else if (wgs(64, 128) >= 256 && d.N % 128 == 0) code = 19;
    else code = 20;
  }
  const GemmTile* t = nullptr;
  for (const GemmTile& e : GEMM_TILES)
    if (e.code == code) t = &e;
  if (!t) return nullptr;
  const unsigned f = t->flags;
  if (geglu && !(f & TILE_GEGLU)) return nullptr;
  if (t->loop == LOOP_DMA8 && (d.K % BK)) return nullptr;
  if ((t->loop == LOOP_PIPE || t->loop == LOOP_PHASE) && ((d.K % BK) || (ga.cin % BK) || (d.c0 % BK))) return nullptr;
  if ((f & TILE_PLAIN) && (d.taps != 1 || d.c1 > 0)) return nullptr;
  if (t->loop == LOOP_PHASE) {
    if (d.c1 > 0 || d.nb_o * d.nb_i != 1) return nullptr;
    if (((long)d.M + 2L * d.win + 2) * d.lda0 * 2 + 2L * d.K >= (1L << 31) || (long)d.N * d.ldw * 2 >= (1L << 31))
      return nullptr;
  }
  if ((f & TILE_CONV_SAME) && d.taps == 9 && (d.stride != 1 || d.ups != 0 || d.hin != d.hout || d.win != d.wout))
    return nullptr;
  if ((f & TILE_ONE_SPLIT) && d.splits != 1) return nullptr;
  if ((f & TILE_LDS_EPI) && d.splits == 1) {
    const long c_off_max = (long)(d.nb_o - 1) * d.c_bs_o + (long)(d.nb_i - 1) * d.c_bs_i;
    if ((d.epi & LGD_EPI_OUT_F32) || (d.N & 7) || (d.ldc & 7) || (c_off_max & 7) || (d.c_bs_o & 7) || (d.c_bs_i & 7) ||
        (reinterpret_cast<uintptr_t>(d.c) & 15) || (d.res && (d.epi & (LGD_EPI_RES_F32 | LGD_EPI_GEGLU))))
      return nullptr;
  }
  if (d.splits > 1 && d.cnt && !(f & TILE_CNT)) return nullptr;
  return t;
}

using GemmKernel = void (*)(GemmArgs);

int lds_kernel(GemmKernel kern, int smem, int threads, long* resident = nullptr) {
  static std::mutex mu;
  static std::map<std::pair<GemmKernel, int>, long> ready;
  int dev = 0;
  if (hipGetDevice(&dev) != hipSuccess) return LGD_ERR_LAUNCH;
  std::lock_guard<std::mutex> lock(mu);
  auto it = ready.find({kern, dev});
  if (it == ready.end()) {
    if (hipFuncSetAttribute(reinterpret_cast<const void*>(kern), hipFuncAttributeMaxDynamicSharedMemorySize, smem) !=
        hipSuccess)
      return LGD_ERR_LAUNCH;
    it = ready.emplace(std::make_pair(kern, dev), -1L).first;
  }
  if (resident) {
    if (it->second < 0) {
      int per_cu = 0, cus = 0;
      if (hipDeviceGetAttribute(&cus, hipDeviceAttributeMultiprocessorCount, dev) != hipSuccess ||
          hipOccupancyMaxActiveBlocksPerMultiprocessor(&per_cu, reinterpret_cast<const void*>(kern), threads, smem) !=
              hipSuccess)
        return LGD_ERR_LAUNCH;
      it->second = (long)(cus / 8) * 8 * (per_cu > 0 ? per_cu : 1);
    }
    *resident = it->second;
  }
  return LGD_OK;
}

template <int MI, int NI, int WM = 2>
int launch_gemm(const GemmArgs& ga, hipStream_t st, bool dma) {
  constexpr int BM = WM * 16 * MI, BN = 32 * NI;
  const LgdGemmDesc& d = ga.d;
  long tiles = (long)((d.M + BM - 1) / BM) * ((d.N + BN - 1) / BN);
  dim3 grid((unsigned)tiles, 1, (unsigned)(d.nb_o * d.nb_i * d.splits));
  if constexpr (WM == 2) {
    if (dma) hipLaunchKernelGGL((gemm_dma_kernel<MI, NI, 2>), grid, dim3(256), 0, st, ga);
    else hipLaunchKernelGGL((gemm_kernel<MI, NI>), grid, dim3(256), 0, st, ga);
  } else {
    hipLaunchKernelGGL((gemm_dma_kernel<MI, NI, WM>), grid, dim3(128 * WM), 0, st, ga);
  }
  return lgd_check_launch();
}

template <int MI, int NI, int WM, int WN, int NS, bool CM>
int launch_gemm_pipe_cm(const GemmArgs& ga, hipStream_t st) {
  constexpr int BM = WM * 16 * MI, BN = WN * 16 * NI;
  constexpr int SMEM = NS * (BM + BN) * BK * 2;
  constexpr int THREADS = 64 * WM * WN;
  constexpr bool HAS_PERSIST = !CM && !(MI == 4 && NI == 5) && NS != 2;
  const LgdGemmDesc& d = ga.d;
  long tiles = (long)((d.M + BM - 1) / BM) * ((d.N + BN - 1) / BN);
  GemmKernel kern = &gemm_pipe_kernel<MI, NI, WM, WN, NS, CM>;
  long resident = 0;
  if constexpr (HAS_PERSIST) {
    static const bool persist_on = [] { const char* e = getenv("LGD_GEMM_PERSIST"); return !(e && e[0] == '0'); }();
    if (persist_on)
      if (int rc = lds_kernel(&gemm_pipe_kernel<MI, NI, WM, WN, NS, false, true>, SMEM, THREADS, &resident)) return rc;
  }
  const bool persist = resident > 0 && d.nb_o * d.nb_i * d.splits == 1 && tiles > resident && d.K <= 10 * BK && d.taps == 1;
  dim3 grid((unsigned)(persist ? resident : tiles), 1, (unsigned)(d.nb_o * d.nb_i * d.splits));
  if constexpr (HAS_PERSIST)
    if (persist) kern = &gemm_pipe_kernel<MI, NI, WM, WN, NS, false, true>;
#ifdef LGD_GEMM_ABLATION
  static const int abl = [] { const char* e = getenv("LGD_GEMM_ABL"); return e ? atoi(e) : 0; }();
  if (abl) {
    switch (abl) {
      case 1: kern = &gemm_pipe_kernel<MI, NI, WM, WN, NS, CM, false, 1>; break;
      case 2: kern = &gemm_pipe_kernel<MI, NI, WM, WN, NS, CM, false, 2>; break;
      case 3: kern = &gemm_pipe_kernel<MI, NI, WM, WN, NS, CM, false, 3>; break;
      case 4: kern = &gemm_pipe_kernel<MI, NI, WM, WN, NS, CM, false, 4>; break;
      case 6: kern = &gemm_pipe_kernel<MI, NI, WM, WN, NS, CM, false, 6>; break;
      case 8: kern = &gemm_pipe_kernel<MI, NI, WM, WN, NS, CM, false, 8>; break;
      case 11: kern = &gemm_pipe_kernel<MI, NI, WM, WN, NS, CM, false, 11>; break;
      case 16: kern = &gemm_pipe_kernel<MI, NI, WM, WN, NS, CM, false, 16>; break;
      case 17: kern = &gemm_pipe_kernel<MI, NI, WM, WN, NS, CM, false, 17>; break;
      case 20: kern = &gemm_pipe_kernel<MI, NI, WM, WN, NS, CM, false, 20>; break;
      default: return lgd_check_launch();
    }
  }
#endif
  if (int rc = lds_kernel(kern, SMEM, THREADS)) return rc;
  hipLaunchKernelGGL(kern, grid, dim3(THREADS), SMEM, st, ga);
  return lgd_check_launch();
}

template <int MI, int NI, int WM, int WN, int NS>
int launch_gemm_pipe(const GemmArgs& ga, hipStream_t st) {
  const LgdGemmDesc& d = ga.d;
  static const int no_cm = [] { const char* e = getenv("LGD_GEMM_NO_CM"); return (e && e[0] == '1') ? 1 : 0; }();
  if constexpr (NS != 2) {
    if (d.taps == 9 && d.stride == 1 && d.ups == 0 && d.c1 == 0 && !no_cm)
      return launch_gemm_pipe_cm<MI, NI, WM, WN, NS, true>(ga, st);
  }
  return launch_gemm_pipe_cm<MI, NI, WM, WN, NS, false>(ga, st);
}

template <int MI, int NI>
int launch_gemm_phase(const GemmArgs& ga, hipStream_t st) {
  constexpr int BM = 32 * MI, BN = 64 * NI;
  constexpr int SMEM = 2 * (BM + BN) * BK * 2;
  const LgdGemmDesc& d = ga.d;
  const bool conv = d.taps == 9;
  long tiles = (long)((d.M + BM - 1) / BM) * ((d.N + BN - 1) / BN);
  dim3 grid((unsigned)tiles, 1, (unsigned)(d.nb_o * d.nb_i * d.splits));
  GemmKernel kern = conv ? &gemm_phase_kernel<MI, NI, true> : &gemm_phase_kernel<MI, NI, false>;
#ifdef LGD_GEMM_ABLATION
  static const int abl = [] { const char* e = getenv("LGD_GEMM_ABL"); return e ? atoi(e) : 0; }();
  if (abl) {
#define LGD_PH_ABL(A) case A: kern = conv ? &gemm_phase_kernel<MI, NI, true, A> : &gemm_phase_kernel<MI, NI, false, A>; break;
    switch (abl) {
      LGD_PH_ABL(1) LGD_PH_ABL(2) LGD_PH_ABL(3) LGD_PH_ABL(4) LGD_PH_ABL(6) LGD_PH_ABL(16) LGD_PH_ABL(17) LGD_PH_ABL(20) LGD_PH_ABL(32) LGD_PH_ABL(64) LGD_PH_ABL(96)
      default: return lgd_check_launch();
    }
#undef LGD_PH_ABL
  }
#endif
  if (int rc = lds_kernel(kern, SMEM, 512)) return rc;
  hipLaunchKernelGGL(kern, grid, dim3(512), SMEM, st, ga);
  return lgd_check_launch();
}

int launch_tile(const GemmTile& t, const GemmArgs& ga, hipStream_t st) {
  const bool dma = t.loop == LOOP_DMA && ga.d.K % BK == 0;
  switch (t.code) {
    case 33: return launch_gemm_pipe<4, 5, 4, 2, 3>(ga, st);
    case 34: return launch_gemm_pipe<4, 4, 4, 2, 3>(ga, st);
    case 35: return launch_gemm_pipe<4, 2, 4, 2, 4>(ga, st);
    case 37: return launch_gemm_pipe<2, 5, 4, 2, 4>(ga, st);
    case 38: return launch_gemm_pipe<2, 4, 4, 2, 4>(ga, st);
    case 39: return launch_gemm_pipe<2, 2, 4, 2, 5>(ga, st);
    case 40: return launch_gemm_pipe<1, 5, 4, 2, 5>(ga, st);
    case 41: return launch_gemm_pipe<1, 4, 4, 2, 5>(ga, st);
    case 42: return launch_gemm_pipe<1, 2, 4, 2, 6>(ga, st);
    case 44: return launch_gemm_pipe<4, 8, 4, 2, 2>(ga, st);
    case 45: return launch_gemm_pipe<2, 4, 4, 2, 2>(ga, st);
    case 46: return launch_gemm_phase<8, 4>(ga, st);
    case 47: return launch_gemm_phase<8, 5>(ga, st);
    case 1: case 17: return launch_gemm<4, 4>(ga, st, dma);
    case 2: case 18: return launch_gemm<4, 2>(ga, st, dma);
    case 3: case 19: return launch_gemm<2, 4>(ga, st, dma);
    case 4: case 20: return launch_gemm<2, 2>(ga, st, dma);
    case 5: case 21: return launch_gemm<1, 4>(ga, st, dma);
    case 6: case 22: return launch_gemm<4, 5>(ga, st, dma);
    case 7: case 23: return launch_gemm<2, 5>(ga, st, dma);
    case 25: return launch_gemm<4, 10, 4>(ga, st, true);
    case 26: return launch_gemm<4, 4, 4>(ga, st, true);
  }
  return LGD_ERR_ARG;
}

}

extern "C" int lgd_abi_version(void) { return LGD_ABI_VERSION; }

extern "C" int lgd_gemm_check(const LgdGemmDesc* desc) {
  GemmArgs ga;
  return desc && gemm_check(*desc, ga) ? LGD_OK : LGD_ERR_ARG;
}

extern "C" int lgd_gemm_f16(const LgdGemmDesc* desc, void* stream) {
  (void)hipGetLastError();
  GemmArgs ga;
  const GemmTile* t = desc ? gemm_check(*desc, ga) : nullptr;
  if (!t) return LGD_ERR_ARG;
  const LgdGemmDesc& d = ga.d;
  hipStream_t st = reinterpret_cast<hipStream_t>(stream);
#ifdef LGD_GEMM_ABLATION
  { const char* e = getenv("LGD_GEMM_STAGGER"); ga.stagger = e ? atoi(e) : 0; }
#endif
  {
    static const int forced = [] { const char* e = getenv("LGD_GEMM_GROUP_M"); return e ? atoi(e) : 0; }();
    ga.group_m = 1;
    const long w_bytes = (long)d.N * d.K * 2;
    if (d.taps == 1 && d.nb_o * d.nb_i == 1 && w_bytes > (5L << 19)) {
      long g = (3L << 20) / (256L * d.K * 2);
      ga.group_m = forced > 0 ? forced : (int)(g < 1 ? 1 : g > 8 ? 8 : g);
    }
  }
  int rc = launch_tile(*t, ga, st);
  if (rc || d.splits == 1 || d.cnt) return rc;
  int n_out = (d.epi & LGD_EPI_GEGLU) ? d.N / 2 : d.N;
  long total = (long)d.M * (n_out / 4);
  int blocks = (int)((total + 255) / 256);
  if (blocks > 2048) blocks = 2048;
  dim3 grid(blocks, 1, d.nb_o * d.nb_i);
  hipLaunchKernelGGL(splitk_reduce_kernel, grid, dim3(256), 0, st, ga);
  return lgd_check_launch();
}
```

llm-groundeddiffusion_amd/csrc/norm.hip:

```cpp
#include "common.h"
#include "../../include/lgd_hip.h"

namespace {

constexpr int GN_MAXC = 4096;

constexpr int GN_PASS_C = 2048;
constexpr int GN_UNROLL = 4;
constexpr int GN_UNROLL_S = 8;

__device__ __forceinline__ void gn_group_reduce(float* s_a, float* s_b, const float (&a)[8],
                                                const float (&b)[8], bool active, int slot, int c_lo,
                                                int c_n, int pl, int cpg, int G, float& acc_a,
                                                float& acc_b) {
  if (active) {
#pragma unroll
    for (int e = 0; e < 8; ++e) { s_a[slot + e] = a[e]; s_b[slot + e] = b[e]; }
  }
  __syncthreads();
  __shared__ float s_tot[64][2];
  int T = 1;
  while (T * 2 * G <= 256 && T < 64) T *= 2;
  {
    const int g = threadIdx.x / T, j = threadIdx.x - g * T;
// ... 787 lines not shown
    const half_t* xr = x + bb * x_bs + (long)rr * ldx;
#pragma unroll
    for (int j = 0; j < V; ++j) {
      const int v = li + j * L;
      h[r][j] = v < nvec ? *reinterpret_cast<const half8_t*>(xr + v * 8) : (half8_t){0, 0, 0, 0, 0, 0, 0, 0};
    }
  }
  const float inv_c = 1.f / C;
  float mean[R], var[R];
#pragma unroll
  for (int r = 0; r < R; ++r) {
    float s = 0.f;
#pragma unroll
    for (int j = 0; j < V; ++j)
#pragma unroll
      for (int e = 0; e < 8; ++e) s += (float)h[r][j][e];
    mean[r] = s;
  }
#pragma unroll
  for (int r = 0; r < R; ++r) mean[r] = lane_group_sum<L>(mean[r]) * inv_c;
#pragma unroll
  for (int r = 0; r < R; ++r)
#pragma unroll
    for (int j = 0; j < V; ++j) asm volatile("" : "+v"(h[r][j]));
#pragma unroll
  for (int r = 0; r < R; ++r) {
    float q = 0.f;
#pragma unroll
    for (int j = 0; j < V; ++j)
      if (li + j * L < nvec) {
#pragma unroll
        for (int e = 0; e < 8; ++e) {
          const float dlt = (float)h[r][j][e] - mean[r];
          q += dlt * dlt;
        }
      }
    var[r] = q;
  }
#pragma unroll
  for (int r = 0; r < R; ++r) var[r] = lane_group_sum<L>(var[r]) * inv_c;
#pragma unroll
  for (int r = 0; r < R; ++r) {
    const int row = row0 + r * RPW;
    if (li == 0 && row < rows) *reinterpret_cast<float2*>(stats + (long)row * 2) = make_float2(mean[r], rsqrtf(var[r] + eps));
  }
}

__global__ __launch_bounds__(256) void layernorm_bwd_kernel(
    const half_t* __restrict__ gy, long ldgy, const half_t* __restrict__ x, long ldx, half_t* gx,
    long ldgx, int rows, int C, const float* __restrict__ gamma, const float* __restrict__ stats,
    int rpb, long gy_bs, long x_bs, long gx_bs, int accumulate) {
  const int lane = threadIdx.x & 63;
  const int row = blockIdx.x * 4 + (threadIdx.x >> 6);
  if (row >= rows) return;
  const int bb = row / rpb, rr = row - bb * rpb;
  const half_t* gr = gy + bb * gy_bs + (long)rr * ldgy;
  const half_t* xr = x + bb * x_bs + (long)rr * ldx;
  half_t* dr = gx + bb * gx_bs + (long)rr * ldgx;
  const float mean = stats[(long)row * 2], rstd = stats[(long)row * 2 + 1];
  const int nvec = C / 8;
  float dxh[LN_MAXV][8], xh[LN_MAXV][8];
  float s1 = 0.f, s2 = 0.f;
#pragma unroll
  for (int j = 0; j < LN_MAXV; ++j) {
    int v = lane + j * 64;
    if (v < nvec) {
      half8_t hx = *reinterpret_cast<const half8_t*>(xr + v * 8);
      half8_t hg = *reinterpret_cast<const half8_t*>(gr + v * 8);
#pragma unroll
      for (int e = 0; e < 8; ++e) {
        float a = ((float)hx[e] - mean) * rstd;
        float d = (float)hg[e] * gamma[v * 8 + e];
        xh[j][e] = a;
        dxh[j][e] = d;
        s1 += d;
        s2 += d * a;
      }
    }
  }
  s1 = wave_sum(s1) / C;
  s2 = wave_sum(s2) / C;
#pragma unroll
  for (int j = 0; j < LN_MAXV; ++j) {
    int v = lane + j * 64;
    if (v < nvec) {
      half8_t o;
      if (accumulate) o = *reinterpret_cast<const half8_t*>(dr + v * 8);
#pragma unroll
      for (int e = 0; e < 8; ++e) {
        float dx = rstd * (dxh[j][e] - s1 - xh[j][e] * s2);
        if (accumulate) dx += (float)o[e];
        o[e] = (half_t)dx;
      }
      *reinterpret_cast<half8_t*>(dr + v * 8) = o;
    }
  }
}

int g_gn_apply_wgs = 1024;
int gn_apply_blocks(int B, int HW, int C) {
  const int nvec = C / 8;
  const int pl = nvec < 256 ? 256 / nvec : 1;
  int px = GN_UNROLL * pl;
  const int want = (int)(((long)HW * B + g_gn_apply_wgs - 1) / g_gn_apply_wgs);
  if (px < want) px = want;
  int n = (HW + px - 1) / px;
  return n < 1 ? 1 : n;
}

}

void lgd_gn_set_fused_hw(int hw) { g_gn_fused_hw = hw; }
void lgd_ln_set_stream(int on) { g_ln_stream = on; }
void lgd_gn_set_slab(int on) { g_gn_slab = on; }
void lgd_gn_set_apply_wgs(int n) { g_gn_apply_wgs = n; }

extern "C" int lgd_groupnorm_f16(const void* x0, const void* x1, int c0, int c1, int B, int HW,
                                 int G, float eps, const float* gamma, const float* beta, int silu,
                                 void* y, float* part, int nchunk, float* stats, void* stream) {
  (void)hipGetLastError();
  const int C = c0 + c1;
  if (G > 64 || C > GN_MAXC || (C % G) || (c0 % 8) || (c1 % 8) || nchunk < 1) return LGD_ERR_ARG;
  if (c1 > 0 && !x1) return LGD_ERR_ARG;
  hipStream_t st = reinterpret_cast<hipStream_t>(stream);
  {
    const int cpg = C / G;
    int kg = 1;
    while ((kg * cpg) % 8) kg *= 2;
    const int W = kg * cpg, nv = W / 8;
    if (HW <= g_gn_fused_hw && kg <= 8 && (G % kg) == 0 && W <= 256) {
      const int pl = 256 / nv, npx = (HW + pl - 1) / pl;
      if (npx <= 32) {
#define GN_FUSED(P)                                                                                                 \
  hipLaunchKernelGGL(gn_fused_kernel<P>, dim3(G / kg, B), dim3(256), 0, st, (const half_t*)x0, (const half_t*)x1,    \
                     c0, c1, HW, G, eps, gamma, beta, silu, (half_t*)y, stats, kg)
        if (npx <= 4) GN_FUSED(4);
        else if (npx <= 8) GN_FUSED(8);
        else if (npx <= 16) GN_FUSED(16);
        else GN_FUSED(32);
#undef GN_FUSED
        return lgd_check_launch();
      }
    }
  }
  hipLaunchKernelGGL(gn_stats_kernel, dim3(nchunk, B), dim3(256), 0, st, (const half_t*)x0,
                     (const half_t*)x1, c0, c1, HW, G, part, nchunk);
  const int napply = gn_apply_blocks(B, HW, C);
  hipLaunchKernelGGL(gn_apply_kernel, dim3(napply, B), dim3(256), 0, st, (const half_t*)x0,
                     (const half_t*)x1, c0, c1, HW, G, eps, gamma, beta, silu, (half_t*)y, part,
                     nchunk, stats, napply);
  return lgd_check_launch();
}

extern "C" int lgd_groupnorm_bwd_f16(const void* gy, const void* x0, const void* x1, int c0, int c1,
                                     int B, int HW, int G, const float* gamma, const float* beta,
                                     int silu, const float* stats, void* gx0, void* gx1, float* part,
                                     int nchunk, int accumulate, void* stream) {
  (void)hipGetLastError();
  const int C = c0 + c1;
  if (G > 64 || C > GN_MAXC || (C % G) || (c0 % 8) || (c1 % 8) || nchunk < 1) return LGD_ERR_ARG;
  hipStream_t st = reinterpret_cast<hipStream_t>(stream);
  {
    int kg, nv;
    if (g_gn_slab && gn_slab_geometry(C, G, kg, nv)) {
#define GN_BWD_SLAB_(NT, P, S)                                                                                      \
  hipLaunchKernelGGL((gn_bwd_slab_kernel<NT, P, S>), dim3(G / kg, B), dim3(NT), 0, st, (const half_t*)gy,             \
                     (const half_t*)x0, (const half_t*)x1, c0, c1, HW, G, gamma, beta, stats, (half_t*)gx0,           \
                     (half_t*)gx1, accumulate, kg)
#define GN_BWD_SLAB(NT, P) do { if (silu) GN_BWD_SLAB_(NT, P, true); else GN_BWD_SLAB_(NT, P, false); } while (0)
      const long slab_bytes = 2L * HW * (8 * nv) * 2;
      if (slab_bytes <= 96 * 1024) {
        if (HW <= 8 * (256 / nv)) { GN_BWD_SLAB(256, 8); return lgd_check_launch(); }
        if (HW <= 11 * (512 / nv)) { GN_BWD_SLAB(512, 11); return lgd_check_launch(); }
      }
#undef GN_BWD_SLAB
#undef GN_BWD_SLAB_
    }
  }
  hipLaunchKernelGGL(gn_bwd_stats_kernel, dim3(nchunk, B), dim3(256), 0, st, (const half_t*)gy,
                     (const half_t*)x0, (const half_t*)x1, c0, c1, HW, G, gamma, beta, silu, stats,
                     part, nchunk);
  const int napply = gn_apply_blocks(B, HW, C);
  hipLaunchKernelGGL(gn_bwd_apply_kernel, dim3(napply, B), dim3(256), 0, st, (const half_t*)gy,
                     (const half_t*)x0, (const half_t*)x1, c0, c1, HW, G, gamma, beta, silu, stats,
                     (half_t*)gx0, (half_t*)gx1, part, nchunk, accumulate, napply);
  return lgd_check_launch();
}

extern "C" int lgd_layernorm_f16(const void* x, int64_t ldx, void* y, int64_t ldy, int rows, int C,
                                 float eps, const float* gamma, const float* beta, float* stats,
                                 int rows_per_batch, int64_t x_bs, int64_t y_bs, void* stream) {
  (void)hipGetLastError();
  if ((C % 8) || C > 64 * 8 * LN_MAXV || rows < 1) return LGD_ERR_ARG;
  if (!y && (!stats || C > (g_ln_stream ? 64 * 5 * 8 : 192 * 8))) return LGD_ERR_ARG;
  if (rows_per_batch < 1) rows_per_batch = rows;
  hipStream_t st = reinterpret_cast<hipStream_t>(stream);
  const half_t* xp = (const half_t*)x;
  half_t* yp = (half_t*)y;
  const int nvec = C / 8;
  if (!y && g_ln_stream && ((long)rows * C >= (8L << 20) || nvec > 192)) {
#define LGD_LN_STATS(L, R)                                                                                         \
  hipLaunchKernelGGL((ln_stats_kernel<L, R>), dim3((rows + 4 * (64 / L) * R - 1) / (4 * (64 / L) * R)), dim3(256), 0, st, xp, \
                     (long)ldx, rows, C, eps, stats, rows_per_batch, (long)x_bs)
    if (nvec <= 40) LGD_LN_STATS(8, 4);
    else if (nvec <= 80) LGD_LN_STATS(16, 4);
    else if (nvec <= 160) LGD_LN_STATS(32, 4);
    else LGD_LN_STATS(64, 2);
#undef LGD_LN_STATS
    return lgd_check_launch();
  }
#define LGD_LN_LAUNCH(MAXV, ROWS)                                                                   \
  hipLaunchKernelGGL((layernorm_rows_kernel<MAXV, ROWS>), dim3((rows + 4 * ROWS - 1) / (4 * ROWS)), \
                     dim3(256), 0, st, xp, (long)ldx, yp, (long)ldy, rows, C, eps, gamma, beta,      \
                     stats, rows_per_batch, (long)x_bs, (long)y_bs)
  if (nvec <= 64) LGD_LN_LAUNCH(1, 4);
  else if (nvec <= 128) LGD_LN_LAUNCH(2, 4);
  else if (nvec <= 192) LGD_LN_LAUNCH(3, 2);
  else
    hipLaunchKernelGGL(layernorm_kernel, dim3((rows + 3) / 4), dim3(256), 0, st, xp, (long)ldx, yp,
                       (long)ldy, rows, C, eps, gamma, beta, stats, rows_per_batch, (long)x_bs,
                       (long)y_bs);
#undef LGD_LN_LAUNCH
  return lgd_check_launch();
}

extern "C" int lgd_layernorm_bwd_f16(const void* gy, int64_t ldgy, const void* x, int64_t ldx,
                                     void* gx, int64_t ldgx, int rows, int C, const float* gamma,
                                     const float* stats, int rows_per_batch, int64_t gy_bs,
                                     int64_t x_bs, int64_t gx_bs, int accumulate, void* stream) {
  (void)hipGetLastError();
  if ((C % 8) || C > 64 * 8 * LN_MAXV || rows < 1 || !stats) return LGD_ERR_ARG;
  if (rows_per_batch < 1) rows_per_batch = rows;
  hipStream_t st = reinterpret_cast<hipStream_t>(stream);
  hipLaunchKernelGGL(layernorm_bwd_kernel, dim3((rows + 3) / 4), dim3(256), 0, st,
                     (const half_t*)gy, (long)ldgy, (const half_t*)x, (long)ldx, (half_t*)gx,
                     (long)ldgx, rows, C, gamma, stats, rows_per_batch, (long)gy_bs, (long)x_bs,
                     (long)gx_bs, accumulate);
  return lgd_check_launch();
}
```

llm-groundeddiffusion_amd/ops.py:

```python
import contextlib
import ctypes as C

import torch

from . import _lib
from ._lib import EPI_GEGLU, EPI_OUT_F32, EPI_RES_F32, EPI_ROWNORM, LgdGemmDesc

F16, F32 = torch.float16, torch.float32


def _stream():
    return C.c_void_p(torch.cuda.current_stream().cuda_stream)


def _p(t):
    return C.c_void_p(t.data_ptr()) if t is not None else C.c_void_p(0)


def _call(name, *args):
    lib = _lib.load()
    rc = getattr(lib, name)(*args)
    _lib.check(rc, name)


def set_option(name: str, value: int):
    _call("lgd_set_option", name.encode(), int(value))


import threading as _threading
_TLS = _threading.local()
WS_FLOATS = 1 << 26


def workspace(device) -> torch.Tensor:
    dev = torch.device(device)
    ws = getattr(_TLS, "ws", None)
    if ws is None or ws.device != dev:
        ws = _TLS.ws = torch.empty(WS_FLOATS, device=dev, dtype=F32)
    return ws


N_COUNTERS = 1 << 16
import os as _os
SPLITK_IN_LAUNCH = _os.environ.get("LGD_SPLITK_IN_LAUNCH", "0") == "1"


def splitk_counters(device):
    dev = torch.device(device)
    cnt = getattr(_TLS, "cnt", None)
    if cnt is None or cnt.device != dev:
        cnt = _TLS.cnt = torch.zeros(N_COUNTERS, device=dev, dtype=torch.int32)
    return cnt


def choose_splits(M, N, K, batches=1):
    wgs = ((M + 127) // 128) * ((N + 63) // 64) * batches
    if wgs >= 256:
        return 1
    ktiles = K // 64
    s = min((512 + wgs - 1) // wgs, max(1, ktiles // 4), 16)
    return max(1, s)


def gemm_desc(a0, w, c, M, N, K, *, a1=None, lda0=None, lda1=0, c0=None, c1=0, taps=1,
              hin=0, win=0, hout=0, wout=0, stride=1, ups=0, ldw=None, bias=None, bias2=None,
              res=None, ldr=0, alpha=1.0, epi=0, ldc=None, splits=None, ws=None, tile=0,
              nb_o=1, nb_i=1, a_bs=(0, 0), w_bs=(0, 0), c_bs=(0, 0), r_bs=(0, 0), rowstat=None, colsum=None):
    d = LgdGemmDesc()
    ptr = lambda t: (t.data_ptr() if torch.is_tensor(t) else (t or 0))
    d.a0, d.a1 = ptr(a0), ptr(a1)
    cin = K // taps
    d.c0 = cin - c1 if c0 is None else c0
    d.c1 = c1
    d.lda0 = d.c0 if lda0 is None else lda0
    d.lda1 = lda1 if lda1 else max(c1, 0)
    d.taps, d.hin, d.win, d.hout, d.wout, d.stride, d.ups = taps, hin, win, hout, wout, stride, ups
    d.w = ptr(w)
    d.ldw = K if ldw is None else ldw
    d.M, d.N, d.K = M, N, K
    d.nb_o, d.nb_i = nb_o, nb_i
    d.a_bs_o, d.a_bs_i = a_bs
    d.w_bs_o, d.w_bs_i = w_bs
    d.c_bs_o, d.c_bs_i = c_bs
    d.r_bs_o, d.r_bs_i = r_bs
    d.bias, d.bias2 = ptr(bias), ptr(bias2)
    d.res, d.ldr = ptr(res), ldr
    if rowstat is not None:
        epi |= EPI_ROWNORM
    d.rowstat, d.colsum = ptr(rowstat), ptr(colsum)
    d.alpha, d.epi = alpha, epi
    d.c = ptr(c)
    n_out = N // 2 if (epi & EPI_GEGLU) else N
    d.ldc = n_out if ldc is None else ldc
    ent = tuning_table().get(shape_key(d)) if (splits is None or not tile) else None
    if splits is None:
        splits = ent["splits"] if ent else choose_splits(M, N, K, nb_o * nb_i)
    if splits > 1 and ws is None:
        need = splits * M * N * nb_o * nb_i
        ws = workspace(c.device if torch.is_tensor(c) else "cuda")
        if need > ws.numel():
            raise RuntimeError(f"split-K workspace too small for {splits}x{M}x{N}")
    d.splits, d.ws = splits, ptr(ws)
    d.cnt = 0
    d.tile = tile
    if not tile:
        if ent and ent["splits"] == splits:
            d.tile = ent["tile"]
        if not d.tile or not gemm_accepts(d):
            d.tile = choose_tile(M, N, nb_o * nb_i * max(splits, 1), bool(epi & EPI_GEGLU), K,
                                 pipe_ok=(K % 64 == 0 and d.c0 % 64 == 0 and d.c1 % 64 == 0))
    log = getattr(_TUNING_TLS, "log", None)
    if log is not None:
        log.append((shape_key(d), d.tile, splits))
    if splits > 1 and SPLITK_IN_LAUNCH and torch.is_tensor(c) and c.is_cuda:
        if nb_o * nb_i * ((M + 31) // 32) * ((N + 63) // 64) <= N_COUNTERS:
            d.cnt = splitk_counters(c.device).data_ptr()
            if not gemm_accepts(d):
                d.cnt = 0
    return d


def gemm_accepts(d) -> bool:
    return _lib.load().lgd_gemm_check(C.byref(d)) == 0


TILE_NAMES = {
    1: "gemm_kernel<4,4> 128x128", 2: "gemm_kernel<4,2> 128x64", 3: "gemm_kernel<2,4> 64x128", 4: "gemm_kernel<2,2> 64x64",
    5: "gemm_kernel<1,4> 32x128", 6: "gemm_kernel<4,5> 128x160", 7: "gemm_kernel<2,5> 64x160",
    17: "gemm_dma_kernel<4,4,2> 128x128", 18: "gemm_dma_kernel<4,2,2> 128x64", 19: "gemm_dma_kernel<2,4,2> 64x128",
    20: "gemm_dma_kernel<2,2,2> 64x64", 21: "gemm_dma_kernel<1,4,2> 32x128", 22: "gemm_dma_kernel<4,5,2> 128x160",
    23: "gemm_dma_kernel<2,5,2> 64x160", 25: "gemm_dma_kernel<4,10,4> 256x320", 26: "gemm_dma_kernel<4,4,4> 256x128",
    33: "gemm_pipe_kernel<4,5,4,2,3> 256x160", 34: "gemm_pipe_kernel<4,4,4,2,3> 256x128",
    35: "gemm_pipe_kernel<4,2,4,2,4> 256x64", 37: "gemm_pipe_kernel<2,5,4,2,4> 128x160",
    38: "gemm_pipe_kernel<2,4,4,2,4> 128x128", 39: "gemm_pipe_kernel<2,2,4,2,5> 128x64",
    40: "gemm_pipe_kernel<1,5,4,2,5> 64x160", 41: "gemm_pipe_kernel<1,4,4,2,5> 64x128",
    42: "gemm_pipe_kernel<1,2,4,2,6> 64x64", 44: "gemm_pipe_kernel<4,8,4,2,2> 256x256",
    45: "gemm_pipe_kernel<2,4,4,2,2> 128x128 x2/CU", 46: "gemm_phase_kernel<8,4> 256x256",
    47: "gemm_phase_kernel<8,5> 256x320",
}


def choose_tile(M, N, batches=1, geglu=False, K=64, pipe_ok=False):
    wgs = lambda bm, bn: batches * ((M + bm - 1) // bm) * ((N + bn - 1) // bn)
    if M <= 32:
        return 21
    if pipe_ok:
        if not geglu and N % 160 == 0 and wgs(256, 160) >= 256:
            return 33
        if N % 128 == 0 and wgs(256, 128) >= 256:
            return 34
        if not geglu and N % 160 == 0 and wgs(128, 160) >= 256:
            return 37
        if N % 128 == 0 and wgs(128, 128) >= 256:
            return 38
    if not geglu and N % 160 == 0:
        if wgs(128, 160) >= 384:
            return 22
        if wgs(64, 160) >= 256:
            return 23
    if wgs(128, 128) >= 384 and N % 128 == 0:
        return 17
    if wgs(64, 128) >= 256 and N % 128 == 0:
        return 19
    return 20


def shape_key(d) -> str:
    return (f"M{d.M}_N{d.N}_K{d.K}_t{d.taps}_c{d.c0}+{d.c1}_h{d.hin}x{d.hout}_s{d.stride}_u{d.ups}"
            f"_e{d.epi & 1}_b{d.nb_o * d.nb_i}")


_TUNING = {}
TUNING_MODE = _os.environ.get("LGD_TUNING_MODE", "latency")
_TUNING_FILES = {"latency": ("tuning_gfx950.json",), "throughput": ("tuning_gfx950.json", "tuning_gfx950_lanes.json"),
                 "heuristic": ()}
_TUNING_TLS = _threading.local()


def set_tuning_mode(mode: str):
    global TUNING_MODE
    if mode not in _TUNING_FILES:
        raise ValueError(f"tuning mode {mode!r}: expected one of {sorted(_TUNING_FILES)}")
    if _os.environ.get("LGD_TUNING_MODE"):
        return
    TUNING_MODE = mode


def current_tuning_mode() -> str:
    if _os.environ.get("LGD_TUNING_MODE"):
        return TUNING_MODE
    return getattr(_TUNING_TLS, "mode", None) or TUNING_MODE


@contextlib.contextmanager
def tuning(mode):
    if mode is not None and mode not in _TUNING_FILES:
        raise ValueError(f"tuning mode {mode!r}: expected one of {sorted(_TUNING_FILES)}")
    prev = getattr(_TUNING_TLS, "mode", None)
    if mode is not None:
        _TUNING_TLS.mode = mode
    try:
        yield
    finally:
        _TUNING_TLS.mode = prev


@contextlib.contextmanager
def desc_log():
    prev, _TUNING_TLS.log = getattr(_TUNING_TLS, "log", None), []
    try:
        yield _TUNING_TLS.log
    finally:
        _TUNING_TLS.log = prev


def tuning_table():
    mode = current_tuning_mode()
    if mode not in _TUNING:
        import json
        tab = {}
        for fname in _TUNING_FILES[mode]:
            path = _os.path.join(_os.path.dirname(_os.path.abspath(__file__)), fname)
            if _os.path.exists(path):
                tab.update(json.load(open(path)))
        _TUNING[mode] = tab
    return _TUNING[mode]


class LaunchProfiler:

    def __init__(self, max_records=20000):
        self.recs = []
        self.max = max_records
        self.enabled = True

    def wrap(self, name, flops, nbytes, fn, tag=None, shape=None):
        if not self.enabled or len(self.recs) >= self.max:
            return fn()
        e0, e1 = torch.cuda.Event(enable_timing=True), torch.cuda.Event(enable_timing=True)
        e0.record()
        r = fn()
        e1.record()
        self.recs.append((name, flops, nbytes, e0, e1, tag, shape))
        return r

    def summary(self, by_tag=False, by_shape=False):
        torch.cuda.synchronize()
        agg = {}
        for name, fl, nb, e0, e1, tag, shape in self.recs:
            if by_tag and tag is None:
                continue
            key = tag if by_tag else (f"{name} | {shape}" if by_shape else name)
            a = agg.setdefault(key, dict(ms=0.0, flops=0.0, bytes=0.0, n=0))
            a["ms"] += e0.elapsed_time(e1)
            a["flops"] += fl
            a["bytes"] += nb
            a["n"] += 1
        return agg


PROFILER = None


def _prof(name, nbytes, fn, *, flops=0.0, tag=None, shape=None):
    if PROFILER is not None:
        return PROFILER.wrap(name, flops, nbytes, fn, tag, shape)
    return fn()


def copy_(dst, src):
    return _prof("copy", 2.0 * dst.numel() * dst.element_size(), lambda: dst.copy_(src))


def zero_(t):
    return _prof("fill", float(t.numel() * t.element_size()), lambda: t.zero_())


def gemm_launch(desc, tag=None, flops=None):
    if PROFILER is not None:
        nb = desc.nb_o * desc.nb_i
        if flops is None:
            flops = 2.0 * desc.M * desc.N * desc.K * nb
        nbytes = 2.0 * nb * (desc.M * desc.K / max(desc.taps, 1) + desc.N * desc.K + desc.M * desc.N)
        return PROFILER.wrap(TILE_NAMES.get(desc.tile, "gemm"), flops, nbytes,
                             lambda: _call("lgd_gemm_f16", C.byref(desc), _stream()), tag,
                             shape=f"{shape_key(desc)} splits={desc.splits}")
    _call("lgd_gemm_f16", C.byref(desc), _stream())


def linear(x, w, bias=None, res=None, out=None, *, alpha=1.0, geglu=False, out_f32=False,
           splits=None, ws=None, tile=0, bias2=None, rowstat=None, colsum=None):
    M, K = x.shape
    N = w.shape[0]
    n_out = N // 2 if geglu else N
    if out is None:
        out = torch.empty((M, n_out), device=x.device, dtype=F32 if out_f32 else F16)
    epi = (EPI_GEGLU if geglu else 0) | (EPI_OUT_F32 if out_f32 else 0)
    if res is not None and res.dtype == F32:
        epi |= EPI_RES_F32
    d = gemm_desc(x, w, out, M, N, K, bias=bias, bias2=bias2, res=res,
                  ldr=(res.stride(0) if res is not None else 0), alpha=alpha, epi=epi,
                  splits=splits, ws=ws, tile=tile, lda0=x.stride(0), ldw=w.stride(0),
                  ldc=out.stride(0), rowstat=rowstat, colsum=colsum)
    gemm_launch(d)
    return out


def conv3x3(x, w, B, H, W, *, x1=None, bias=None, bias2=None, res=None, stride=1, ups=False,
            out=None, splits=None, ws=None, tile=0, alpha=1.0):
    c0 = x.shape[1]
    c1 = x1.shape[1] if x1 is not None else 0
    Cout = w.shape[0]
    K = 9 * (c0 + c1)
    assert w.shape[1] == K
    if ups:
        Hl, Wl = 2 * H, 2 * W
    else:
        Hl, Wl = H, W
    Ho, Wo = (Hl - 1) // stride + 1, (Wl - 1) // stride + 1
    M = B * Ho * Wo
    if out is None:
        out = torch.empty((M, Cout), device=x.device, dtype=F16)
    d = gemm_desc(x, w, out, M, Cout, K, a1=x1, c0=c0, c1=c1, lda0=x.stride(0),
                  lda1=(x1.stride(0) if x1 is not None else 0), taps=9, hin=H, win=W, hout=Ho,
                  wout=Wo, stride=stride, ups=int(ups), bias=bias, bias2=bias2, res=res,
                  ldr=(res.stride(0) if res is not None else 0), splits=splits, ws=ws, tile=tile,
                  alpha=alpha, ldc=out.stride(0))
    gemm_launch(d)
    return out


def conv_in(x_nchw, w, bias, out=None):
    B, Cin, L, _ = x_nchw.shape
    Cout = w.shape[0]
    if out is None:
        out = torch.empty((B * L * L, Cout), device=x_nchw.device, dtype=F16)
    _call("lgd_conv_in_f16", _p(x_nchw), _p(w), _p(bias), _p(out), B, Cin, L, Cout, _stream())
    return out


def nchw_to_nhwc8(x_nchw, out=None):
    B, C_, H, W = x_nchw.shape
    if out is None:
        out = torch.empty((B * H * W, 8), device=x_nchw.device, dtype=F16)
    _prof("nchw_to_nhwc8_kernel", 4.0 * x_nchw.numel() + 2.0 * out.numel(),
          lambda: _call("lgd_nchw_to_nhwc8_f16", _p(x_nchw), _p(out), B, C_, H * W, _stream()))
    return out


def conv_out(x, w, bias, B, L, out=None, out_scale=1.0):
    Cin = x.shape[1]
    Cout = w.shape[0]
    if out is None:
        out = torch.empty((B, Cout, L, L), device=x.device, dtype=F32)
    _prof("conv_out_kernel", 2.0 * x.numel() + 4.0 * out.numel(),
          lambda: _call("lgd_conv_out_f16", _p(x), _p(w), _p(bias), _p(out), B, Cin, L, Cout, float(out_scale), _stream()),
          flops=2.0 * B * L * L * Cout * 9 * Cin)
    return out


GN_STATS_WGS = int(_os.environ.get("LGD_GN_STATS_WGS", "1024"))


def gn_chunks(B, HW):
    return max(1, min(HW // 8, GN_STATS_WGS // max(B, 1), 64))


def groupnorm(x, B, HW, G, eps, gamma, beta, silu, *, x1=None, out=None, part=None, stats=None):
    c0 = x.shape[1]
    c1 = x1.shape[1] if x1 is not None else 0
    C_ = c0 + c1
    nchunk = gn_chunks(B, HW)
    if out is None:
        out = torch.empty((B * HW, C_), device=x.device, dtype=F16)
    if part is None:
        part = torch.empty((B, nchunk, G, 2), device=x.device, dtype=F32)
    _prof("groupnorm (gn_stats + gn_apply | gn_fused)", 6.0 * B * HW * C_,
          lambda: _call("lgd_groupnorm_f16", _p(x), _p(x1), c0, c1, B, HW, G, float(eps), _p(gamma), _p(beta),
                        1 if silu else 0, _p(out), _p(part), nchunk, _p(stats), _stream()), shape=f"B{B}_HW{HW}_C{C_}")
    return out


def groupnorm_bwd(gy, x, B, HW, G, gamma, beta, silu, stats, *, x1=None, gx0=None, gx1=None,
                  part=None, accumulate=False):
    c0 = x.shape[1]
    c1 = x1.shape[1] if x1 is not None else 0
    nchunk = gn_chunks(B, HW)
    if gx0 is None:
        gx0 = torch.empty_like(x)
    if x1 is not None and gx1 is None:
        gx1 = torch.empty_like(x1)
    if part is None:
        part = torch.empty((B, nchunk, G, 2), device=x.device, dtype=F32)
    _prof("groupnorm_bwd (gn_bwd_stats + gn_bwd_apply)", (10.0 + (2.0 if accumulate else 0.0)) * B * HW * (c0 + c1),
          lambda: _call("lgd_groupnorm_bwd_f16", _p(gy), _p(x), _p(x1), c0, c1, B, HW, G, _p(gamma), _p(beta),
                        1 if silu else 0, _p(stats), _p(gx0), _p(gx1), _p(part), nchunk, 1 if accumulate else 0, _stream()),
          shape=f"B{B}_HW{HW}_C{c0 + c1}")
    return gx0, gx1


def layernorm(x, gamma, beta, eps=1e-5, *, out=None, ldy=None, stats=None, rows_per_batch=0,
              x_bs=0, y_bs=0, rows=None, ldx=None):
    C_ = gamma.shape[0]
    if rows is None:
        rows = x.numel() // C_
    if out is None:
        out = torch.empty((rows, C_), device=x.device, dtype=F16)
    _prof("layernorm_rows_kernel", 4.0 * rows * C_,
          lambda: _call("lgd_layernorm_f16", _p(x), ldx or C_, _p(out), ldy or C_, rows, C_, float(eps), _p(gamma),
                        _p(beta), _p(stats), rows_per_batch, x_bs, y_bs, _stream()), shape=f"R{rows}_C{C_}")
    return out


def layernorm_stats(x, C_, eps=1e-5, *, stats=None, rows=None, ldx=None):
    if rows is None:
        rows = x.numel() // C_
    if stats is None:
        stats = torch.empty((rows, 2), device=x.device, dtype=torch.float32)
    _prof("ln_stats_kernel (LayerNorm statistics only)", 2.0 * rows * C_,
          lambda: _call("lgd_layernorm_f16", _p(x), ldx or C_, _p(None), C_, rows, C_, float(eps), _p(None), _p(None),
                        _p(stats), 0, 0, 0, _stream()), shape=f"R{rows}_C{C_}")
    return stats


def layernorm_bwd(gy, x, gamma, stats, *, gx=None, rows=None, ldgy=None, ldx=None, ldgx=None,
                  rows_per_batch=0, gy_bs=0, x_bs=0, gx_bs=0, accumulate=False):
    C_ = gamma.shape[0]
    if rows is None:
        rows = x.numel() // C_
    if gx is None:
        gx = torch.empty((rows, C_), device=x.device, dtype=F16)
    _prof("layernorm_bwd_kernel", (6.0 + (2.0 if accumulate else 0.0)) * rows * C_,
          lambda: _call("lgd_layernorm_bwd_f16", _p(gy), ldgy or C_, _p(x), ldx or C_, _p(gx), ldgx or C_, rows, C_,
                        _p(gamma), _p(stats), rows_per_batch, gy_bs, x_bs, gx_bs, 1 if accumulate else 0, _stream()),
          shape=f"R{rows}_C{C_}")
    return gx


def attn_fwd(q, k, v, o, B, H, Sq, Sk, d, scale, *, lse=None, q_view=None, k_view=None,
             v_view=None, o_view=None):
    qv = q_view or (H * d, Sq * H * d)
    kv = k_view or (H * d, Sk * H * d)
    vv = v_view or (H * d, Sk * H * d)
    ov = o_view or (H * d, Sq * H * d)
    fn = lambda: _call("lgd_attn_fwd_f16", _p(q), qv[0], qv[1], _p(k), kv[0], kv[1], _p(v), vv[0], vv[1],
                       _p(o), ov[0], ov[1], _p(lse), B, H, Sq, Sk, d, float(scale), _stream())
    if PROFILER is not None:
        PROFILER.wrap(f"attn_self_kernel d={d}", 4.0 * B * H * Sq * Sk * d, 2.0 * B * H * d * (2 * Sq + 2 * Sk), fn,
                      "attn_path", shape=f"B{B}_H{H}_Sq{Sq}_Sk{Sk}")
    else:
        fn()
    return o


def attn_bwd(q, k, v, o, go, lse, delta, gq, gk, gv, B, H, Sq, Sk, d, scale, *, q_view=None,
             k_view=None, v_view=None, o_view=None, go_view=None, gq_view=None, gk_view=None,
             gv_view=None, sk_grad=None):
    skg = Sk if sk_grad is None else int(sk_grad)
    dq_ = (H * d, Sq * H * d)
    dk_ = (H * d, Sk * H * d)
    qv, kv, vv = q_view or dq_, k_view or dk_, v_view or dk_
    ov, gov = o_view or dq_, go_view or dq_
    gqv, gkv, gvv = gq_view or dq_, gk_view or dk_, gv_view or dk_
    _prof(f"attn_bwd_dq + attn_bwd_dkv d={d}", 2.0 * B * H * d * (4 * Sq + 4 * Sk),
          lambda: _call("lgd_attn_bwd_keys_f16", _p(q), qv[0], qv[1], _p(k), kv[0], kv[1], _p(v), vv[0], vv[1], _p(o),
                        ov[0], ov[1], _p(go), gov[0], gov[1], _p(lse), _p(delta), _p(gq), gqv[0], gqv[1], _p(gk),
                        gkv[0], gkv[1], _p(gv), gvv[0], gvv[1], B, H, Sq, Sk, skg, d, float(scale), _stream()),
          flops=6.0 * B * H * Sq * Sk * d + 4.0 * B * H * Sq * skg * d, tag="attn_path_bwd", shape=f"B{B}_H{H}_Sq{Sq}_Sk{Sk}")


def cross_attn_fwd(q, k, v, o, B, H, Sq, Sk, d, scale, *, probs=None, tok=-1, cond_only=False,
                   q_view=None, k_view=None, v_view=None, o_view=None):
    qv = q_view or (H * d, Sq * H * d)
    kv = k_view or (H * d, Sk * H * d)
    vv = v_view or (H * d, Sk * H * d)
    ov = o_view or (H * d, Sq * H * d)
    fn = lambda: _call("lgd_cross_attn_fwd_f16", _p(q), qv[0], qv[1], _p(k), kv[0], kv[1], _p(v), vv[0], vv[1],
                       _p(o), ov[0], ov[1], _p(probs), int(tok), 1 if cond_only else 0, B, H, Sq, Sk, d,
                       float(scale), _stream())
    if PROFILER is not None:
        PROFILER.wrap(f"attn_fwd_kernel(cross) d={d}", 4.0 * B * H * Sq * Sk * d,
                      2.0 * B * H * d * (2 * Sq + 2 * Sk), fn, "attn_path")
    else:
        fn()
    return o


def attn_causal_fwd(q, k, v, o, B, H, S, d, scale, *, view=None):
    vw = view or (H * d, S * H * d)
    _call("lgd_attn_causal_fwd_f16", _p(q), vw[0], vw[1], _p(k), vw[0], vw[1], _p(v), vw[0], vw[1], _p(o),
          H * d, S * H * d, B, H, S, d, float(scale), _stream())
    return o


def quick_gelu(x, out=None):
    if out is None:
        out = torch.empty_like(x)
    _call("lgd_quick_gelu_f16", _p(x), _p(out), x.numel(), _stream())
    return out


ACT_GELU, ACT_RELU = 1, 2


def act(x, mode, out=None):
    if out is None:
        out = torch.empty_like(x)
    _call("lgd_act_f16", _p(x), _p(out), x.numel(), int(mode), _stream())
    return out


def sam_relpos_qkv(qkv, qkv_bias, rel_h, rel_w, B, Hs, Ws, window, NH, d, DA, scale):
    S = window or Hs
    rows = B * (-(-Hs // S)) * (-(-Ws // S)) * S * S
    qa, ka, va = (torch.empty((rows, NH * DA), device=qkv.device, dtype=F16) for _ in range(3))
    _call("lgd_sam_relpos_qkv_f16", _p(qkv), _p(qkv_bias), _p(rel_h), _p(rel_w), B, Hs, Ws, window, NH, d, DA,
          float(scale), _p(qa), _p(ka), _p(va), _stream())
    return qa, ka, va


def sam_window_merge(oa, B, Hs, Ws, window, NH, d, DA):
    out = torch.empty((B * Hs * Ws, NH * d), device=oa.device, dtype=F16)
    _call("lgd_sam_window_merge_f16", _p(oa), _p(out), B, Hs, Ws, window, NH, d, DA, _stream())
    return out


def cross_attn_bwd(q, k, v, go, gp, gq, B, H, Sq, Sk, d, scale, *, q_view=None, k_view=None,
                   v_view=None, go_view=None, gq_view=None):
    dq_ = (H * d, Sq * H * d)
    dk_ = (H * d, Sk * H * d)
    qv, kv, vv = q_view or dq_, k_view or dk_, v_view or dk_
    gov, gqv = go_view or dq_, gq_view or dq_
# ... 111 lines not shown
```

llm-groundeddiffusion_amd/unet.py:

```python
import math
import os
from collections import OrderedDict
from typing import Dict, List, Optional, Sequence, Tuple

import torch

from . import ops
from ._lib import EPI_GEGLU
from .weights import UNetConfig, unet_blocks
from .weightstore import WeightStore

F16, F32 = torch.float16, torch.float32
N_OBJ_TOKENS = 30


class Act:
    __slots__ = ("t", "g", "rows", "C")

    def __init__(self, t):
        self.t = t
        self.g = None
        self.rows, self.C = t.shape


class Op:
    def __init__(self, fwd, make_bwd=None, gouts=(), passthrough=None):
        self.fwd = fwd
        self.make_bwd = make_bwd
        self.gouts = list(gouts)
        self.acc = None
        self.bwd = None
        self.passthrough = passthrough


choose_splits = ops.choose_splits


class Plan:
    def __init__(self, eng: "UNetEngine", B: int, L: int, *, grad: bool, fuser: bool,
                 stop_key: Optional[Tuple] = None, save_keys: Sequence[Tuple] = (),
                 text_batch_offset: int = 0, obj_batch_offset: int = 0):
        self.eng, self.B, self.L = eng, B, L
        self.obj_off = obj_batch_offset
        self.grad, self.fuser = grad, fuser
        self.stop_key = tuple(stop_key) if stop_key else None
        self.save_keys = [tuple(k) for k in save_keys]
        self.text_off = text_batch_offset
        self.ops: List[Op] = []
        self._buffers: List[torch.Tensor] = []
        self.dbg: Dict[str, Act] = {}
        self.maps: Dict[Tuple, torch.Tensor] = {}
        self.gmaps: Dict[Tuple, torch.Tensor] = {}
        self._cursor = [0, 0]
        self.arena_bytes = 0
        self.latents_in = self._alloc((B, eng.cfg.in_channels, L, L))
        self.eps_out = None
        self.g_latents = None
        self._build()

    def _new(self, rows, C, dtype=F16):
        return self._alloc((rows, C), dtype)

    def _alloc(self, shape, dtype=F32):
        t, self._cursor = self.eng.arena_take(self._cursor, shape, dtype)
        self.arena_bytes += t.numel() * t.element_size()
        self._buffers.append(t)
        return t

    def _act(self, rows, C):
        return Act(self._new(rows, C))

    def _add(self, fwd, make_bwd=None, gouts=(), passthrough=None):
        self.ops.append(Op(fwd, make_bwd if self.grad else None, gouts if self.grad else (),
                           passthrough if self.grad else None))

    def _ws(self, n_floats):
        return self.eng.workspace(n_floats)

    def linear(self, x: Act, name: str, *, res: Optional[Act] = None, alpha=1.0, geglu=False,
               bias=True, out: Optional[Act] = None, rows=None, bwd=True) -> Act:
        W = self.eng.w.h[f"{name}.w"]
        b = self.eng.w.f[f"{name}.b"] if bias else None
        N, K = W.shape
        M = rows or x.rows
        n_out = N // 2 if geglu else N
        y = out or self._act(M, n_out)
        d = ops.gemm_desc(x.t, W, y.t, M, N, K, lda0=x.C, bias=b, res=res.t if res else None,
                          ldr=res.C if res else 0, alpha=alpha, epi=EPI_GEGLU if geglu else 0,
                          ldc=y.C)
        tag = "attn_path" if any(t in name for t in (".attn1.", ".attn2.", ".fuser.attn.")) else None
        fwd = lambda: ops.gemm_launch(d, tag)
        if not (self.grad and bwd):
            self._add(fwd)
            return y
        assert not geglu, "grad plans keep the GEGLU pre-activation (see ff())"
        Wt = self.eng.w.h[f"{name}.wt"]
        gouts = [x] + ([res] if res else [])

        def make_bwd(acc):
            dd = ops.gemm_desc(y.g, Wt, x.g, M, K, N, lda0=y.C, alpha=alpha, ldc=x.C,
                               res=x.g if acc[0] else None, ldr=x.C)
            if res is None:
                return lambda: ops.gemm_launch(dd)
            racc = acc[1]
            aliased = res.g.data_ptr() == y.g.data_ptr()

            def run():
                ops.gemm_launch(dd)
                if racc:
                    ops.add(res.g, y.g, res.g)
                elif not aliased:
                    ops.copy_(res.g, y.g)
            return run
        self._add(fwd, make_bwd, gouts, passthrough=(res, y) if res is not None else None)
        return y

    def conv(self, x: Act, name: str, H: int, *, x1: Optional[Act] = None, res: Optional[Act] = None,
             temb_off: Optional[int] = None, stride=1, ups=False) -> Act:
        B = self.B
        W = self.eng.w.h[f"{name}.w"]
        b = self.eng.w.f[f"{name}.b"]
        Cout, K = W.shape
        c0, c1 = x.C, (x1.C if x1 else 0)
        Hl = 2 * H if ups else H
        Ho = (Hl - 1) // stride + 1
        M = B * Ho * Ho
        y = self._act(M, Cout)
        eng = self.eng
        if temb_off is not None and eng.temb_rows > 1:
            assert stride == 1 and not ups and res is None
            ds = []
            for i in range(B):
                row = eng.temb_cur[self.text_off + i]
                sl = slice(i * H * H, (i + 1) * H * H)
                ds.append(ops.gemm_desc(x.t[sl], W, y.t[sl], H * H, Cout, K, a1=x1.t[sl] if x1 else None, c0=c0, c1=c1,
                                        lda0=c0, lda1=c1, taps=9, hin=H, win=H, hout=H, wout=H, bias=b,
                                        bias2=row[temb_off:temb_off + Cout], ldc=Cout))
            fwd = lambda: [ops.gemm_launch(dd) for dd in ds]
        else:
            bias2 = eng.temb_cur[0, temb_off:temb_off + Cout] if temb_off is not None else None
            d = ops.gemm_desc(x.t, W, y.t, M, Cout, K, a1=x1.t if x1 else None, c0=c0, c1=c1, lda0=c0,
                              lda1=c1, taps=9, hin=H, win=H, hout=Ho, wout=Ho, stride=stride,
                              ups=1 if ups else 0, bias=b, bias2=bias2, res=res.t if res else None,
                              ldr=res.C if res else 0, ldc=Cout)
            fwd = lambda: ops.gemm_launch(d)
        if not self.grad:
            self._add(fwd)
            return y
        Wd = self.eng.w.h[f"{name}.wd"]
        gouts = [x] + ([x1] if x1 else []) + ([res] if res else [])

        def make_bwd(acc):
            runs = []
            Kd = 9 * Cout
            if stride == 1 and not ups:
                for i, (src, lo, cn) in enumerate([(x, 0, c0)] + ([(x1, c0, c1)] if x1 else [])):
                    dd = ops.gemm_desc(y.g, Wd[lo:lo + cn], src.g, src.rows, cn, Kd, c0=Cout, lda0=Cout,
                                       taps=9, hin=H, win=H, hout=H, wout=H, ldc=cn,
                                       res=src.g if acc[i] else None, ldr=cn)
                    runs.append(lambda dd=dd: ops.gemm_launch(dd))
            elif stride == 2:
                dd = ops.gemm_desc(y.g, Wd, x.g, x.rows, c0, Kd, c0=Cout, lda0=Cout, taps=9, hin=Ho,
                                   win=Ho, hout=H, wout=H, ups=2, ldc=c0,
                                   res=x.g if acc[0] else None, ldr=c0)
                runs.append(lambda: ops.gemm_launch(dd))
            else:
                tmp = self._new(B * Hl * Hl, c0)
                dd = ops.gemm_desc(y.g, Wd, tmp, B * Hl * Hl, c0, Kd, c0=Cout, lda0=Cout, taps=9,
                                   hin=Hl, win=Hl, hout=Hl, wout=Hl, ldc=c0)
                assert not acc[0]
                runs.append(lambda: (ops.gemm_launch(dd), ops.upsample2x_bwd(tmp, B, H, H, c0, out=x.g)))
            if res is not None:
                racc = acc[-1]
                if racc:
                    runs.append(lambda: ops.add(res.g, y.g, res.g))
                elif res.g.data_ptr() != y.g.data_ptr():
                    runs.append(lambda: ops.copy_(res.g, y.g))
            return lambda: [r() for r in runs]
        self._add(fwd, make_bwd, gouts, passthrough=(res, y) if res is not None else None)
        return y

    def shortcut(self, x: Act, x1: Optional[Act], name: str) -> Act:
        W = self.eng.w.h[f"{name}.w"]
        b = self.eng.w.f[f"{name}.b"]
        Cout, K = W.shape
        c0, c1 = x.C, (x1.C if x1 else 0)
        M = x.rows
        y = self._act(M, Cout)
        d = ops.gemm_desc(x.t, W, y.t, M, Cout, K, a1=x1.t if x1 else None, c0=c0, c1=c1, lda0=c0,
                          lda1=c1, bias=b, ldc=Cout)
        fwd = lambda: ops.gemm_launch(d)
        if not self.grad:
            self._add(fwd)
            return y
        Wt = self.eng.w.h[f"{name}.wt"]
        gouts = [x] + ([x1] if x1 else [])

        def make_bwd(acc):
            runs = []
            for i, (src, lo, cn) in enumerate([(x, 0, c0)] + ([(x1, c0, c1)] if x1 else [])):
                dd = ops.gemm_desc(y.g, Wt[lo:lo + cn], src.g, M, cn, Cout, lda0=Cout, ldc=cn,
                                   res=src.g if acc[i] else None, ldr=cn)
                runs.append(lambda dd=dd: ops.gemm_launch(dd))
            return lambda: [r() for r in runs]
        self._add(fwd, make_bwd, gouts)
        return y

    def groupnorm(self, x: Act, x1: Optional[Act], name: str, HW: int, eps: float, silu: bool) -> Act:
        eng, B = self.eng, self.B
        G = eng.cfg.norm_num_groups
        gm, bt = eng.w.f[f"{name}.g"], eng.w.f[f"{name}.b"]
        C = x.C + (x1.C if x1 else 0)
        y = self._act(x.rows, C)
        nch = ops.gn_chunks(B, HW)
        part = self._alloc((B, nch, G, 2))
        stats = self._alloc((B, G, 2)) if self.grad else None
        xt1 = x1.t if x1 else None
        fwd = lambda: ops.groupnorm(x.t, B, HW, G, eps, gm, bt, silu, x1=xt1, out=y.t, part=part, stats=stats)
        if not self.grad:
            self._add(fwd)
            return y
        gouts = [x] + ([x1] if x1 else [])

        def make_bwd(acc):
            a = acc[0]
            if x1 is not None:
                assert acc[0] == acc[1], "mixed accumulate modes on a concat GroupNorm"
            return lambda: ops.groupnorm_bwd(y.g, x.t, B, HW, G, gm, bt, silu, stats, x1=xt1, gx0=x.g,
                                             gx1=x1.g if x1 else None, part=part, accumulate=a)
        self._add(fwd, make_bwd, gouts)
        return y

    def layernorm(self, x: Act, name: str, *, out_t=None, ldy=None, S=None, y_bs=0) -> Act:
        eng = self.eng
        gm, bt = eng.w.f[f"{name}.g"], eng.w.f[f"{name}.b"]
        C = x.C
        y = Act(out_t) if out_t is not None else self._act(x.rows, C)
        stats = self._alloc((x.rows, 2)) if self.grad else None
        rpb = S or 0
        x_bs = (S or 0) * C
        fwd = lambda: ops.layernorm(x.t, gm, bt, out=y.t, ldy=ldy or C, stats=stats, rows=x.rows,
                                    rows_per_batch=rpb, x_bs=x_bs, y_bs=y_bs)
        if not self.grad:
            self._add(fwd)
            return y

        def make_bwd(acc):
            return lambda: ops.layernorm_bwd(y.g, x.t, gm, stats, gx=x.g, rows=x.rows, ldgy=ldy or C,
                                             rows_per_batch=rpb, gy_bs=y_bs, x_bs=x_bs, gx_bs=x_bs,
                                             accumulate=acc[0])
        self._add(fwd, make_bwd, [x])
        return y

    def ln_linear(self, x: Act, norm: str, name: str, *, geglu=False) -> Act:
        eng = self.eng
        has_b = f"{name}.b" in eng.w.f
        if self.grad or not eng.fold_ln or x.C > 1536:
            y = self.layernorm(x, norm)
            if geglu:
                return self.linear(y, name, geglu=True)
            return self.linear(y, name, bias=has_b)
        W, cs, b = eng.w.h[f"{name}.wln"], eng.w.f[f"{name}.cs"], eng.w.f[f"{name}.bln"]
        N, K = W.shape
        M = x.rows
        stats = self._alloc((M, 2))
        y = self._act(M, N // 2 if geglu else N)
        d = ops.gemm_desc(x.t, W, y.t, M, N, K, lda0=x.C, bias=b, epi=EPI_GEGLU if geglu else 0, ldc=y.C,
                          rowstat=stats, colsum=cs)
        tag = "attn_path" if any(t in name for t in (".attn1.", ".attn2.", ".fuser.attn.")) else None
        xt = x.t
        self._add(lambda: (ops.layernorm_stats(xt, K, stats=stats, rows=M), ops.gemm_launch(d, tag)))
        return y

    def self_attn(self, qkv: Act, heads: int, S: int, Sk: Optional[int] = None) -> Act:
        B = self.B
        Sk = Sk or S
        C = qkv.C // 3
        d = C // heads
        o = self._act(B * S, C)
        view = (3 * C, Sk * 3 * C)
        lse = self._alloc((B, heads, S)) if self.grad else None
        scale = d ** -0.5
        qt, kt, vt = qkv.t, qkv.t[:, C:], qkv.t[:, 2 * C:]
        fwd = lambda: ops.attn_fwd(qt, kt, vt, o.t, B, heads, S, Sk, d, scale, lse=lse,
                                   q_view=view, k_view=view, v_view=view)
        if not self.grad:
            self._add(fwd)
            return o

        def make_bwd(acc):
            assert not acc[0]
            delta = self._alloc((B, heads, S))
            g = qkv.g
            gq, gk, gv = g, g[:, C:], g[:, 2 * C:]
            pad = Sk > S

            g_tail = g.view(B, Sk, 3 * C)[:, S:, :] if pad else None

            def run():
                if pad:
                    ops.zero_(g_tail)
                ops.attn_bwd(qt, kt, vt, o.t, o.g, lse, delta, gq, gk, gv, B, heads, S, Sk, d, scale,
                             q_view=view, k_view=view, v_view=view, gq_view=view, gk_view=view, gv_view=view, sk_grad=S)
            return run
        self._add(fwd, make_bwd, [qkv])
        return o

    def cross_attn(self, q: Act, key: Tuple, layer_name: str, heads: int, S: int, last: bool) -> Optional[Act]:
        eng, B = self.eng, self.B
        C = q.C
        d = C // heads
        T = eng.text_len
        kv = eng.text_kv[layer_name]
        kv_t = kv[self.text_off:]
        k_view = (2 * C, T * 2 * C)
        o = self._act(B * S, C)
        scale = d ** -0.5
        probs = None
        if key in self.save_keys:
            probs = self.maps[key] = self._alloc((B, heads, S, T))
            if self.grad:
                self.gmaps[key] = self._alloc((B, heads, S, T))
        kt, vt = kv_t, kv_t[:, :, C:]

        def fwd():
            ops.cross_attn_fwd(q.t, kt, vt, o.t, B, heads, S, T, d, scale, probs=probs,
                               k_view=k_view, v_view=k_view)
        if not self.grad:
            self._add(fwd)
            return o
        gp = self.gmaps.get(key)

        def make_bwd(acc):
            assert not acc[0]
            return lambda: ops.cross_attn_bwd(q.t, kt, vt, None if last else o.g, gp, q.g, B, heads, S, T,
                                              d, scale, k_view=k_view, v_view=k_view)
        self._add(fwd, make_bwd, [q])
        return o

    def ff(self, x: Act, res: Act, name: str, alpha=1.0, norm: Optional[str] = None) -> Act:
        if not self.grad:
            h = self.ln_linear(x, norm, f"{name}.net.0.proj", geglu=True) if norm else self.linear(x, f"{name}.net.0.proj", geglu=True)
            return self.linear(h, f"{name}.net.2", res=res, alpha=alpha)
        if norm:
            x = self.layernorm(x, norm)
        pre = self.linear(x, f"{name}.net.0.proj")
        act = self._act(x.rows, pre.C // 2)
        self._add(lambda: ops.geglu_fwd(pre.t, out=act.t),
                  lambda acc: (lambda: ops.geglu_bwd(pre.t, act.g, pre.g)), [pre])
        return self.linear(act, f"{name}.net.2", res=res, alpha=alpha)

    def _resnet(self, r, x: Act, skip: Optional[Act], H: int) -> Act:
        eng = self.eng
        eps = eng.cfg.norm_eps
        HW = H * H
        h = self.groupnorm(x, skip, f"{r.prefix}.norm1", HW, eps, True)
        h = self.conv(h, f"{r.prefix}.conv1", H, temb_off=eng.w.temb_offsets[r.prefix])
        h = self.groupnorm(h, None, f"{r.prefix}.norm2", HW, eps, True)
        if r.shortcut:
            sc = self.shortcut(x, skip, f"{r.prefix}.conv_shortcut")
        else:
            assert skip is None
            sc = x
        out = self.conv(h, f"{r.prefix}.conv2", H, res=sc)
        self.dbg[f"{r.prefix}.out"] = out
        return out

    def _transformer(self, a, x: Act, H: int) -> Optional[Act]:
        eng, B = self.eng, self.B
        S = H * H
        C, heads = a.channels, a.heads
        n = self.groupnorm(x, None, f"{a.prefix}.norm", S, 1e-6, False)
        h = self.linear(n, f"{a.prefix}.proj_in")
        for dpt in range(a.depth):
            t = f"{a.prefix}.transformer_blocks.{dpt}"
            key = tuple(a.key[:3]) + (dpt,)
            qkv = self.ln_linear(h, f"{t}.norm1", f"{t}.attn1.qkv")
            h = self.linear(self.self_attn(qkv, heads, S), f"{t}.attn1.to_out.0", res=h)
            if dpt == 0:
                self.dbg[f"{a.prefix}.after_attn1"] = h
            if self.fuser:
                f = f"{t}.fuser"
                Sk = S + N_OBJ_TOKENS
                cat = eng.fuser_cat(eng.kv_name(a.prefix, dpt), B, S, self.obj_off)
                cat_act = self.layernorm(h, f"{f}.norm1", out_t=cat, ldy=C, S=S, y_bs=Sk * C)
                qkv_f = self.linear(cat_act, f"{f}.attn.qkv", bias=False)
                o = self.self_attn(qkv_f, heads, S, Sk)
                h = self.linear(o, f"{f}.attn.to_out.0", res=h, alpha=eng.w.scalars[f"{f}.alpha_attn"])
                self.dbg[f"{a.prefix}.after_fuser_attn"] = h
                h = self.ff(h, h, f"{f}.ff", alpha=eng.w.scalars[f"{f}.alpha_dense"], norm=f"{f}.norm2")
                self.dbg[f"{a.prefix}.after_fuser"] = h
            q = self.ln_linear(h, f"{t}.norm2", f"{t}.attn2.to_q")
            last = self.stop_key is not None and key == self.stop_key
            o = self.cross_attn(q, key, eng.kv_name(a.prefix, dpt), heads, S, last)
            if last:
                return None
            h = self.linear(o, f"{t}.attn2.to_out.0", res=h)
            if dpt == 0:
                self.dbg[f"{a.prefix}.after_attn2"] = h
            h = self.ff(h, h, f"{t}.ff", norm=f"{t}.norm3")
        out = self.linear(h, f"{a.prefix}.proj_out", res=x)
        self.dbg[f"{a.prefix}.out"] = out
        return out

    def _build(self):
        eng, B, L = self.eng, self.B, self.L
        cfg = eng.cfg
        w = eng.w
        blocks = eng.blocks
        c0 = cfg.block_out_channels[0]
        x = self._act(B * L * L, c0)
        lat = self.latents_in
        self._x0 = x
        x0 = x
        lat8 = self._new(B * L * L, 8)
        d_in = ops.gemm_desc(lat8, w.h["conv_in.w8"], x0.t, B * L * L, c0, 72, c0=8, lda0=8, taps=9, hin=L, win=L, hout=L,
                             wout=L, bias=w.f["conv_in.b"], ldc=c0, splits=1)
        f_in = 2.0 * B * L * L * c0 * 9 * cfg.in_channels
        self._add(lambda: (ops.nchw_to_nhwc8(lat, out=lat8), ops.gemm_launch(d_in, None, f_in)))
        skips = [(x, L)]
        H = L
        done = False
        for b in blocks:
            if done:
                break
            if b.kind == "down":
                for j, r in enumerate(b.resnets):
                    x = self._resnet(r, x, None, H)
                    if b.attns:
                        x = self._transformer(b.attns[j], x, H)
                        if x is None:
                            done = True
                            break
                    skips.append((x, H))
                if done:
                    break
                if b.sampler:
                    x = self.conv(x, b.sampler, H, stride=2)
                    H = (H - 1) // 2 + 1
                    skips.append((x, H))
            elif b.kind == "mid":
                x = self._resnet(b.resnets[0], x, None, H)
                x = self._transformer(b.attns[0], x, H)
                if x is None:
                    done = True
                    break
                x = self._resnet(b.resnets[1], x, None, H)
            else:
                for j, r in enumerate(b.resnets):
                    sk, _ = skips.pop()
                    x = self._resnet(r, x, sk, H)
                    if b.attns:
                        x = self._transformer(b.attns[j], x, H)
                        if x is None:
                            done = True
                            break
                if done:
                    break
                if b.sampler:
                    x = self.conv(x, b.sampler, H, ups=True)
                    H *= 2
        if not done:
            n = self.groupnorm(x, None, "conv_norm_out", H * H, cfg.norm_eps, True)
            self.eps_out = self._alloc((B, cfg.out_channels, L, L))
            eo = self.eps_out
            self._add(lambda: ops.conv_out(n.t, w.h["conv_out.w"], w.f["conv_out.b"], B, L, out=eo))
        if self.grad:
            self._finalize_backward()

    def _finalize_backward(self):
        seen = set()
        for op in reversed(self.ops):
            if op.make_bwd is None:
                continue
            op.acc = []
            for a in op.gouts:
                if a.g is None:
                    pt = op.passthrough
                    if pt is not None and a is pt[0] and pt[1].g is not None and pt[1].g.shape == a.t.shape \
                            and os.environ.get("LGD_RES_GRAD_ALIAS", "1") != "0":
                        a.g = pt[1].g
                    else:
                        a.g = self._alloc(tuple(a.t.shape), a.t.dtype)
                op.acc.append(id(a) in seen)
                seen.add(id(a))
        for op in self.ops:
            if op.make_bwd is not None:
                op.bwd = op.make_bwd(op.acc)
        self.g_latents = self._alloc(tuple(self.latents_in.shape))
        self._bwd_ops = [op.bwd for op in reversed(self.ops) if op.bwd is not None]

    def forward(self, latents: Optional[torch.Tensor] = None):
        if latents is not None:
            self.latents_in.copy_(latents)
        for op in self.ops:
            op.fwd()
        return self.eps_out

    def backward(self, grad_scale: float = 1.0) -> torch.Tensor:
        for b in self._bwd_ops:
            b()
        eng = self.eng
        x0 = self._x0
# ... 195 lines not shown
```

Before: 1.956.

## Compute GroupNorm partial statistics in producer GEMM epilogue

```diff
diff --git a/include/lgd_hip.h b/include/lgd_hip.h
--- a/include/lgd_hip.h
+++ b/include/lgd_hip.h
@@ -44,6 +44,8 @@
 
 int lgd_gemm_f16(const LgdGemmDesc* desc , void* stream);
 int lgd_gemm_check(const LgdGemmDesc* desc );
+int lgd_gemm_gn_check(const LgdGemmDesc* desc , int hw, int cpg);
+int lgd_gemm_gn_f16(const LgdGemmDesc* desc , float* part, int hw, int cpg, void* stream);
 
 int lgd_conv_in_f16(const float* x_nchw, const void* w, const float* bias, void* y, int B, int Cin,
                     int L, int Cout, void* stream);
@@ -53,6 +55,9 @@
 int lgd_groupnorm_f16(const void* x0, const void* x1, int c0, int c1, int B, int HW, int G,
                       float eps, const float* gamma, const float* beta, int silu, void* y,
                       float* part, int nchunk, float* stats, void* stream);
+int lgd_groupnorm_part_f16(const void* x, int C, int B, int HW, int G, float eps, const float* gamma,
+                           const float* beta, int silu, void* y, const float* part, int nchunk, float* stats,
+                           void* stream);
 int lgd_groupnorm_bwd_f16(const void* gy, const void* x0, const void* x1, int c0, int c1, int B,
                           int HW, int G, const float* gamma, const float* beta, int silu,
                           const float* stats, void* gx0, void* gx1, float* part, int nchunk,
diff --git a/llm-groundeddiffusion_amd/_lib.py b/llm-groundeddiffusion_amd/_lib.py
--- a/llm-groundeddiffusion_amd/_lib.py
+++ b/llm-groundeddiffusion_amd/_lib.py
@@ -42,9 +42,12 @@
     "lgd_set_option": [C.c_char_p, _I],
     "lgd_gemm_f16": [C.POINTER(LgdGemmDesc), _P],
     "lgd_gemm_check": [C.POINTER(LgdGemmDesc)],
+    "lgd_gemm_gn_check": [C.POINTER(LgdGemmDesc), _I, _I],
+    "lgd_gemm_gn_f16": [C.POINTER(LgdGemmDesc), _P, _I, _I, _P],
     "lgd_conv_in_f16": [_P, _P, _P, _P, _I, _I, _I, _I, _P],
     "lgd_conv_out_f16": [_P, _P, _P, _P, _I, _I, _I, _I, _F, _P],
     "lgd_groupnorm_f16": [_P, _P, _I, _I, _I, _I, _I, _F, _P, _P, _I, _P, _P, _I, _P, _P],
+    "lgd_groupnorm_part_f16": [_P, _I, _I, _I, _I, _F, _P, _P, _I, _P, _P, _I, _P, _P],
     "lgd_groupnorm_bwd_f16": [_P, _P, _P, _I, _I, _I, _I, _I, _P, _P, _I, _P, _P, _P, _P, _I, _I, _P],
     "lgd_layernorm_f16": [_P, _L, _P, _L, _I, _I, _F, _P, _P, _P, _I, _L, _L, _P],
     "lgd_layernorm_bwd_f16": [_P, _L, _P, _L, _P, _L, _I, _I, _P, _P, _I, _L, _L, _L, _I, _P],
diff --git a/llm-groundeddiffusion_amd/csrc/attn.hip b/llm-groundeddiffusion_amd/csrc/attn.hip
--- a/llm-groundeddiffusion_amd/csrc/attn.hip
+++ b/llm-groundeddiffusion_amd/csrc/attn.hip
@@ -967,6 +967,7 @@
 void lgd_gn_set_slab(int on);
 void lgd_ln_set_stream(int on);
 void lgd_gn_set_apply_wgs(int n);
+void lgd_gemm_set_norm_stats_epi(int on);
 
 extern "C" int lgd_set_option(const char* name, int value) {
   if (!name) return LGD_ERR_ARG;
@@ -974,6 +975,7 @@
   if (!strcmp(name, "gn_slab") && (value == 0 || value == 1)) { lgd_gn_set_slab(value); return LGD_OK; }
   if (!strcmp(name, "ln_stream") && (value == 0 || value == 1)) { lgd_ln_set_stream(value); return LGD_OK; }
   if (!strcmp(name, "gn_apply_wgs") && value >= 64 && value <= 8192) { lgd_gn_set_apply_wgs(value); return LGD_OK; }
+  if (!strcmp(name, "norm_stats_epi") && (value == 0 || value == 1)) { lgd_gemm_set_norm_stats_epi(value); return LGD_OK; }
   if (!strcmp(name, "attn32")) { g_attn32 = value; return LGD_OK; }
   if (!strcmp(name, "attn_w4") && value >= 0 && value <= 2) { g_attn_w4.store(value, std::memory_order_relaxed); return LGD_OK; }
   if (!strcmp(name, "attn_w4_pipe") && (value == 0 || value == 1)) { lgd_attn_w4_set_pipe(value); return LGD_OK; }
diff --git a/llm-groundeddiffusion_amd/csrc/gemm.hip b/llm-groundeddiffusion_amd/csrc/gemm.hip
--- a/llm-groundeddiffusion_amd/csrc/gemm.hip
+++ b/llm-groundeddiffusion_amd/csrc/gemm.hip
@@ -15,6 +15,8 @@
   int cin;
   int k_per_split;
   int group_m;
+  float* gn_part;
+  int gn_hw, gn_cpg;
 #ifdef LGD_GEMM_ABLATION
   int stagger;
 #endif
@@ -335,11 +337,13 @@
   }
 }
 
-template <int MI, int NI, int WM, int WN, int STAGE_B, bool GEGLU, bool RES_PREFETCH, bool RES16, bool RN>
+template <int MI, int NI, int WM, int WN, int STAGE_B, bool GEGLU, bool RES_PREFETCH, bool RES16, bool RN,
+          bool GNS = false>
 __device__ __forceinline__ void gemm_epilogue_lds(const GemmArgs& ga, f32x4 (&acc)[NI][MI], int m0, int n0, int wm,
                                                   int wn, int lane, int tid, long c_off, long r_off,
                                                   unsigned char* lds) {
   static_assert(!(GEGLU && RES16), "GEGLU outputs take no residual here");
+  static_assert(!GNS || (!GEGLU && !RN && RES_PREFETCH), "GroupNorm statistics: plain outputs of one-tile workgroups");
   const LgdGemmDesc& d = ga.d;
   constexpr int NT = 64 * WM * WN;
   constexpr int BM = WM * 16 * MI, BN = WN * 16 * NI;
@@ -405,6 +409,8 @@
     hi += (f32x2_t){b.z, b.w};
   };
   unsigned char* lw = lds + (wm * WROWS + m_l) * CROW + (wn * 16 * NI_OUT + n_l) * 2;
+  static_assert(!GNS || RROWS * CROW + NT * 8 <= STAGE_B, "GroupNorm partials behind the staged rows");
+  float2* gn_red = reinterpret_cast<float2*>(lds + RROWS * CROW);
 #pragma unroll
   for (int r = 0; r < R; ++r) {
     if constexpr (RN && LEAN2) {
@@ -487,9 +493,40 @@
         *reinterpret_cast<uint4*>(cbase + (long)m * d.ldc + n) = val;
       }
     }
-    if (r + 1 < R || !RES_PREFETCH) {
+    if constexpr (GNS) {
+      const int cpg = ga.gn_cpg, lg = __builtin_ctz(BN_OUT / cpg);
+      const unsigned char* gp = lds + (tid & ((1 << lg) - 1)) * cpg * 2;
+      float2 sq = r ? gn_red[tid] : make_float2(0.f, 0.f);
+#pragma unroll 1
+      for (int row = tid >> lg; row < RROWS; row += NT >> lg) {
+        const half2_t* p = reinterpret_cast<const half2_t*>(gp + row * CROW);
+#pragma unroll 1
+        for (int e = 0; e < cpg / 2; ++e) {
+          const half2_t h = p[e];
+          const float x0 = (float)h[0], x1 = (float)h[1];
+          sq.x += x0 + x1;
+          sq.y += x0 * x0 + x1 * x1;
+        }
+      }
+      gn_red[tid] = sq;
+    }
+    if (r + 1 < R || !RES_PREFETCH || GNS) {
       asm volatile("s_waitcnt lgkmcnt(0)" ::: "memory");
       __builtin_amdgcn_s_barrier();
+    }
+  }
+  if constexpr (GNS) {
+    const int cpg = ga.gn_cpg, ng = BN_OUT / cpg;
+    if (tid < ng) {
+      float s = 0.f, q = 0.f;
+      for (int k = 0; k < NT / ng; ++k) {
+        const float2 v = gn_red[k * ng + tid];
+        s += v.x;
+        q += v.y;
+      }
+      const int img = m0 / ga.gn_hw, chunk = (m0 - img * ga.gn_hw) / BM;
+      float* o = ga.gn_part + (((long)img * (ga.gn_hw / BM) + chunk) * (d.N / cpg) + n0_out / cpg + tid) * 2;
+      *reinterpret_cast<float2*>(o) = make_float2(s, q);
     }
   }
 }
@@ -1236,9 +1273,10 @@
       }
       if (lds_epi) {
         unsigned char* free_stage = reinterpret_cast<unsigned char*>(smem) + so_iss;
-#define LGD_EPI_LDS(G, RS, RNORM) \
-  gemm_epilogue_lds<MI, NI, WM, WN, STAGE_B, G, !PERSIST, RS, RNORM>(ga, acc, m0_, n0_, wm, wn, lane, tid, c_off, r_off, free_stage)
+#define LGD_EPI_LDS(G, RS, RNORM, ...) \
+  gemm_epilogue_lds<MI, NI, WM, WN, STAGE_B, G, !PERSIST, RS, RNORM, ##__VA_ARGS__>(ga, acc, m0_, n0_, wm, wn, lane, tid, c_off, r_off, free_stage)
         const bool rn_ = d.epi & LGD_EPI_ROWNORM;
+        const bool gns_ = !PERSIST && ga.gn_part;
         if constexpr (MI * NI >= 32) {
           if (d.epi & LGD_EPI_GEGLU)
             gemm_epilogue_lds_generic<MI, NI, WM, WN, STAGE_B, true, !PERSIST>(ga, acc, m0_, n0_, wm, wn, lane, tid, c_off, r_off, free_stage);
@@ -1249,9 +1287,13 @@
             if (rn_) LGD_EPI_LDS(true, false, true); else LGD_EPI_LDS(true, false, false);
           }
         } else if (d.res) {
-          if (rn_) LGD_EPI_LDS(false, true, true); else LGD_EPI_LDS(false, true, false);
+          if (rn_) LGD_EPI_LDS(false, true, true);
+          else if (gns_) { if constexpr (!PERSIST) LGD_EPI_LDS(false, true, false, true); }
+          else LGD_EPI_LDS(false, true, false);
         } else {
-          if (rn_) LGD_EPI_LDS(false, false, true); else LGD_EPI_LDS(false, false, false);
+          if (rn_) LGD_EPI_LDS(false, false, true);
+          else if (gns_) { if constexpr (!PERSIST) LGD_EPI_LDS(false, false, false, true); }
+          else LGD_EPI_LDS(false, false, false);
         }
 #undef LGD_EPI_LDS
       } else {
@@ -1646,6 +1688,8 @@
 
 const GemmTile* gemm_check(const LgdGemmDesc& desc, GemmArgs& ga) {
   ga.d = desc;
+  ga.gn_part = nullptr;
+  ga.gn_hw = ga.gn_cpg = 0;
   LgdGemmDesc& d = ga.d;
   if (d.M <= 0 || d.N <= 0 || d.K <= 0) return nullptr;
   if (d.taps != 1 && d.taps != 9) return nullptr;
@@ -1709,6 +1753,24 @@
   return t;
 }
 
+int g_norm_stats_epi = 1;
+
+const GemmTile* gemm_gn_check(const LgdGemmDesc& desc, int hw, int cpg, GemmArgs& ga) {
+  const GemmTile* t = gemm_check(desc, ga);
+  if (!t || !g_norm_stats_epi) return nullptr;
+  const LgdGemmDesc& d = ga.d;
+  if (t->loop != LOOP_PIPE || t->bm * t->bn >= 256 * 256) return nullptr;
+  if (d.splits != 1 || d.nb_o * d.nb_i != 1 ||
+      (d.epi & (LGD_EPI_GEGLU | LGD_EPI_ROWNORM | LGD_EPI_OUT_F32 | LGD_EPI_RES_F32)))
+    return nullptr;
+  if ((d.N & 7) || (d.ldc & 7) || (reinterpret_cast<uintptr_t>(d.c) & 15)) return nullptr;
+  if (cpg <= 0 || (cpg & 1) || (t->bn % cpg) || (d.N % t->bn) || (512 % (t->bn / cpg))) return nullptr;
+  if (hw <= 0 || (hw % t->bm) || (d.M % hw)) return nullptr;
+  ga.gn_hw = hw;
+  ga.gn_cpg = cpg;
+  return t;
+}
+
 using GemmKernel = void (*)(GemmArgs);
 
 int lds_kernel(GemmKernel kern, int smem, int threads, long* resident = nullptr) {
@@ -1768,7 +1830,8 @@
     if (persist_on)
       if (int rc = lds_kernel(&gemm_pipe_kernel<MI, NI, WM, WN, NS, false, true>, SMEM, THREADS, &resident)) return rc;
   }
-  const bool persist = resident > 0 && d.nb_o * d.nb_i * d.splits == 1 && tiles > resident && d.K <= 10 * BK && d.taps == 1;
+  const bool persist = resident > 0 && d.nb_o * d.nb_i * d.splits == 1 && tiles > resident && d.K <= 10 * BK && d.taps == 1 &&
+                       !ga.gn_part;
   dim3 grid((unsigned)(persist ? resident : tiles), 1, (unsigned)(d.nb_o * d.nb_i * d.splits));
   if constexpr (HAS_PERSIST)
     if (persist) kern = &gemm_pipe_kernel<MI, NI, WM, WN, NS, false, true>;
@@ -1860,20 +1923,7 @@
   return LGD_ERR_ARG;
 }
 
-}
-
-extern "C" int lgd_abi_version(void) { return LGD_ABI_VERSION; }
-
-extern "C" int lgd_gemm_check(const LgdGemmDesc* desc) {
-  GemmArgs ga;
-  return desc && gemm_check(*desc, ga) ? LGD_OK : LGD_ERR_ARG;
-}
-
-extern "C" int lgd_gemm_f16(const LgdGemmDesc* desc, void* stream) {
-  (void)hipGetLastError();
-  GemmArgs ga;
-  const GemmTile* t = desc ? gemm_check(*desc, ga) : nullptr;
-  if (!t) return LGD_ERR_ARG;
+int gemm_run(const GemmTile* t, GemmArgs& ga, void* stream) {
   const LgdGemmDesc& d = ga.d;
   hipStream_t st = reinterpret_cast<hipStream_t>(stream);
 #ifdef LGD_GEMM_ABLATION
@@ -1898,3 +1948,36 @@
   hipLaunchKernelGGL(splitk_reduce_kernel, grid, dim3(256), 0, st, ga);
   return lgd_check_launch();
 }
+
+}
+
+void lgd_gemm_set_norm_stats_epi(int on) { g_norm_stats_epi = on; }
+
+extern "C" int lgd_abi_version(void) { return LGD_ABI_VERSION; }
+
+extern "C" int lgd_gemm_check(const LgdGemmDesc* desc) {
+  GemmArgs ga;
+  return desc && gemm_check(*desc, ga) ? LGD_OK : LGD_ERR_ARG;
+}
+
+extern "C" int lgd_gemm_gn_check(const LgdGemmDesc* desc, int hw, int cpg) {
+  GemmArgs ga;
+  return desc && gemm_gn_check(*desc, hw, cpg, ga) ? LGD_OK : LGD_ERR_ARG;
+}
+
+extern "C" int lgd_gemm_f16(const LgdGemmDesc* desc, void* stream) {
+  (void)hipGetLastError();
+  GemmArgs ga;
+  const GemmTile* t = desc ? gemm_check(*desc, ga) : nullptr;
+  if (!t) return LGD_ERR_ARG;
+  return gemm_run(t, ga, stream);
+}
+
+extern "C" int lgd_gemm_gn_f16(const LgdGemmDesc* desc, float* gn_part, int hw, int cpg, void* stream) {
+  (void)hipGetLastError();
+  GemmArgs ga;
+  const GemmTile* t = desc && gn_part ? gemm_gn_check(*desc, hw, cpg, ga) : nullptr;
+  if (!t) return LGD_ERR_ARG;
+  ga.gn_part = gn_part;
+  return gemm_run(t, ga, stream);
+}
diff --git a/llm-groundeddiffusion_amd/csrc/norm.hip b/llm-groundeddiffusion_amd/csrc/norm.hip
--- a/llm-groundeddiffusion_amd/csrc/norm.hip
+++ b/llm-groundeddiffusion_amd/csrc/norm.hip
@@ -963,6 +963,18 @@
   return lgd_check_launch();
 }
 
+extern "C" int lgd_groupnorm_part_f16(const void* x, int C, int B, int HW, int G, float eps, const float* gamma,
+                                      const float* beta, int silu, void* y, const float* part, int nchunk, float* stats,
+                                      void* stream) {
+  (void)hipGetLastError();
+  if (G > 64 || C > GN_MAXC || (C % G) || (C % 8) || nchunk < 1 || !part) return LGD_ERR_ARG;
+  hipStream_t st = reinterpret_cast<hipStream_t>(stream);
+  const int napply = gn_apply_blocks(B, HW, C);
+  hipLaunchKernelGGL(gn_apply_kernel, dim3(napply, B), dim3(256), 0, st, (const half_t*)x, (const half_t*)nullptr, C, 0,
+                     HW, G, eps, gamma, beta, silu, (half_t*)y, part, nchunk, stats, napply);
+  return lgd_check_launch();
+}
+
 extern "C" int lgd_groupnorm_bwd_f16(const void* gy, const void* x0, const void* x1, int c0, int c1,
                                      int B, int HW, int G, const float* gamma, const float* beta,
                                      int silu, const float* stats, void* gx0, void* gx1, float* part,
diff --git a/llm-groundeddiffusion_amd/ops.py b/llm-groundeddiffusion_amd/ops.py
--- a/llm-groundeddiffusion_amd/ops.py
+++ b/llm-groundeddiffusion_amd/ops.py
@@ -124,6 +124,14 @@
     return _lib.load().lgd_gemm_check(C.byref(d)) == 0
 
 
+def gemm_gn_accepts(d, hw, cpg) -> bool:
+    return _lib.load().lgd_gemm_gn_check(C.byref(d), int(hw), int(cpg)) == 0
+
+
+def tile_rows(code) -> int:
+    return int(TILE_NAMES[code].split()[1].split("x")[0])
+
+
 TILE_NAMES = {
     1: "gemm_kernel<4,4> 128x128", 2: "gemm_kernel<4,2> 128x64", 3: "gemm_kernel<2,4> 64x128", 4: "gemm_kernel<2,2> 64x64",
     5: "gemm_kernel<1,4> 32x128", 6: "gemm_kernel<4,5> 128x160", 7: "gemm_kernel<2,5> 64x160",
@@ -276,7 +284,17 @@
     return _prof("fill", float(t.numel() * t.element_size()), lambda: t.zero_())
 
 
-def gemm_launch(desc, tag=None, flops=None):
+def gemm_launch(desc, tag=None, flops=None, gn=None):
+    if gn is not None:
+        part, hw, cpg = gn
+        run = lambda: _call("lgd_gemm_gn_f16", C.byref(desc), _p(part), hw, cpg, _stream())
+        if PROFILER is None:
+            return run()
+        nb = desc.nb_o * desc.nb_i
+        flops = 2.0 * desc.M * desc.N * desc.K * nb if flops is None else flops
+        nbytes = 2.0 * nb * (desc.M * desc.K / max(desc.taps, 1) + desc.N * desc.K + desc.M * desc.N)
+        return PROFILER.wrap(TILE_NAMES.get(desc.tile, "gemm"), flops, nbytes, run, tag,
+                             shape=f"{shape_key(desc)} splits={desc.splits}")
     if PROFILER is not None:
         nb = desc.nb_o * desc.nb_i
         if flops is None:
@@ -362,6 +380,9 @@
 GN_STATS_WGS = int(_os.environ.get("LGD_GN_STATS_WGS", "1024"))
 
 
+GN_FUSED_HW = 256
+
+
 def gn_chunks(B, HW):
     return max(1, min(HW // 8, GN_STATS_WGS // max(B, 1), 64))
 
@@ -378,6 +399,16 @@
     _prof("groupnorm (gn_stats + gn_apply | gn_fused)", 6.0 * B * HW * C_,
           lambda: _call("lgd_groupnorm_f16", _p(x), _p(x1), c0, c1, B, HW, G, float(eps), _p(gamma), _p(beta),
                         1 if silu else 0, _p(out), _p(part), nchunk, _p(stats), _stream()), shape=f"B{B}_HW{HW}_C{C_}")
+    return out
+
+
+def groupnorm_part(x, B, HW, G, eps, gamma, beta, silu, part, nchunk, *, out=None, stats=None):
+    C_ = x.shape[1]
+    if out is None:
+        out = torch.empty((B * HW, C_), device=x.device, dtype=F16)
+    _prof("groupnorm (gn_apply on producer statistics)", 4.0 * B * HW * C_,
+          lambda: _call("lgd_groupnorm_part_f16", _p(x), C_, B, HW, G, float(eps), _p(gamma), _p(beta), 1 if silu else 0,
+                        _p(out), _p(part), nchunk, _p(stats), _stream()), shape=f"B{B}_HW{HW}_C{C_}")
     return out
 
 
diff --git a/llm-groundeddiffusion_amd/unet.py b/llm-groundeddiffusion_amd/unet.py
--- a/llm-groundeddiffusion_amd/unet.py
+++ b/llm-groundeddiffusion_amd/unet.py
@@ -15,12 +15,21 @@
 
 
 class Act:
-    __slots__ = ("t", "g", "rows", "C")
+    __slots__ = ("t", "g", "rows", "C", "prod")
 
     def __init__(self, t):
         self.t = t
         self.g = None
         self.rows, self.C = t.shape
+        self.prod = None
+
+
+class Producer:
+    __slots__ = ("d", "gn")
+
+    def __init__(self, d):
+        self.d = d
+        self.gn = None
 
 
 class Op:
@@ -52,6 +61,7 @@
         self.maps: Dict[Tuple, torch.Tensor] = {}
         self.gmaps: Dict[Tuple, torch.Tensor] = {}
         self._cursor = [0, 0]
+        self.norm_paths: Dict[str, int] = {"gn_producer": 0, "gn_stats": 0, "gn_fused": 0}
         self.arena_bytes = 0
         self.latents_in = self._alloc((B, eng.cfg.in_channels, L, L))
         self.eps_out = None
@@ -89,7 +99,10 @@
                           ldr=res.C if res else 0, alpha=alpha, epi=EPI_GEGLU if geglu else 0,
                           ldc=y.C)
         tag = "attn_path" if any(t in name for t in (".attn1.", ".attn2.", ".fuser.attn.")) else None
-        fwd = lambda: ops.gemm_launch(d, tag)
+        prod = Producer(d)
+        if out is None and rows is None:
+            y.prod = prod
+        fwd = lambda: ops.gemm_launch(d, tag, gn=prod.gn)
         if not (self.grad and bwd):
             self._add(fwd)
             return y
@@ -143,7 +156,8 @@
                               lda1=c1, taps=9, hin=H, win=H, hout=Ho, wout=Ho, stride=stride,
                               ups=1 if ups else 0, bias=b, bias2=bias2, res=res.t if res else None,
                               ldr=res.C if res else 0, ldc=Cout)
-            fwd = lambda: ops.gemm_launch(d)
+            prod = y.prod = Producer(d)
+            fwd = lambda: ops.gemm_launch(d, gn=prod.gn)
         if not self.grad:
             self._add(fwd)
             return y
@@ -189,7 +203,8 @@
         y = self._act(M, Cout)
         d = ops.gemm_desc(x.t, W, y.t, M, Cout, K, a1=x1.t if x1 else None, c0=c0, c1=c1, lda0=c0,
                           lda1=c1, bias=b, ldc=Cout)
-        fwd = lambda: ops.gemm_launch(d)
+        prod = y.prod = Producer(d)
+        fwd = lambda: ops.gemm_launch(d, gn=prod.gn)
         if not self.grad:
             self._add(fwd)
             return y
@@ -216,7 +231,14 @@
         part = self._alloc((B, nch, G, 2))
         stats = self._alloc((B, G, 2)) if self.grad else None
         xt1 = x1.t if x1 else None
-        fwd = lambda: ops.groupnorm(x.t, B, HW, G, eps, gm, bt, silu, x1=xt1, out=y.t, part=part, stats=stats)
+        gn = self._producer_stats(x, x1, B, HW, G)
+        if gn is not None:
+            epart, enchunk = gn
+            self.norm_paths["gn_producer"] += 1
+            fwd = lambda: ops.groupnorm_part(x.t, B, HW, G, eps, gm, bt, silu, epart, enchunk, out=y.t, stats=stats)
+        else:
+            self.norm_paths["gn_fused" if HW <= ops.GN_FUSED_HW else "gn_stats"] += 1
+            fwd = lambda: ops.groupnorm(x.t, B, HW, G, eps, gm, bt, silu, x1=xt1, out=y.t, part=part, stats=stats)
         if not self.grad:
             self._add(fwd)
             return y
@@ -349,6 +371,21 @@
         self._add(lambda: ops.geglu_fwd(pre.t, out=act.t),
                   lambda acc: (lambda: ops.geglu_bwd(pre.t, act.g, pre.g)), [pre])
         return self.linear(act, f"{name}.net.2", res=res, alpha=alpha)
+
+    def _producer_stats(self, x: Act, x1: Optional[Act], B: int, HW: int, G: int):
+        p = x.prod
+        if x1 is not None or p is None or HW <= ops.GN_FUSED_HW or x.rows != B * HW or x.C % G:
+            return None
+        cpg = x.C // G
+        if p.gn is None:
+            if not ops.gemm_gn_accepts(p.d, HW, cpg):
+                return None
+            nchunk = HW // ops.tile_rows(p.d.tile)
+            p.gn = (self._alloc((B, nchunk, G, 2)), HW, cpg)
+        part, hw, c = p.gn
+        if (hw, c) != (HW, cpg):
+            return None
+        return part, part.shape[1]
 
     def _resnet(self, r, x: Act, skip: Optional[Act], H: int) -> Act:
         eng = self.eng
```

New measurement: 1.955 (median of 4 runs). Within noise of the previous version (-0.0%).
